# thangktran/HardwareAwareOptimalQuantumCircuitCuttingAndKnitting

Hardware: AMD Instinct MI355X
Metric: subcircuit-instances/s (full-knit wall time = ms_per_step), syc 32 p=2 (higher is better)
Workload: dtype f64

## Files before the change

hardwareawareoptimalquantumcircuitcuttingandknitting_amd/_lib.py:

```python
from __future__ import annotations

import ctypes
import os
import threading

_HERE = os.path.dirname(os.path.abspath(__file__))
LIB_PATH = os.environ.get("QKNIT_LIB") or os.path.join(_HERE, "libqknit.so")

c_i32, c_i64, c_u32, c_u64 = ctypes.c_int32, ctypes.c_int64, ctypes.c_uint32, ctypes.c_uint64
c_vp, c_dp, c_lp = ctypes.c_void_p, ctypes.POINTER(ctypes.c_double), ctypes.POINTER(ctypes.c_int64)


class QkPass(ctypes.Structure):
    _fields_ = [("tile_mask", c_u64), ("group_begin", c_i32), ("group_end", c_i32),
                ("flags", c_i32), ("traced_local", c_u32)]


class QkProgram(ctypes.Structure):
    _fields_ = [("n", c_i32), ("n_eff", c_i32), ("m", c_i32), ("n_slots", c_i32),
                ("packed", c_i32), ("n_passes", c_i32), ("passes", ctypes.POINTER(QkPass)),
                ("ops", c_vp), ("groups", c_vp), ("mats", c_vp)]


class QkLowrankPlan(ctypes.Structure):
    _fields_ = [("nbits", c_i32), ("terms", c_i32), ("rows_a", c_i64), ("rows_b", c_i64), ("mask_a", c_u64),
                ("mask_b", c_u64), ("wt_a", c_vp), ("wt_b", c_vp), ("probes", c_vp), ("lam_tol", ctypes.c_double),
                ("s_tol", ctypes.c_double), ("s_abs", ctypes.c_double), ("rank_tol", ctypes.c_double),
                ("rank_tol_rel", ctypes.c_double)]


class QkKnitPlan(ctypes.Structure):
    _fields_ = [("n_frag", c_i32), ("nbits", c_i32), ("terms", c_i64), ("rows", ctypes.POINTER(c_i64)),
                ("clbit_masks", ctypes.POINTER(c_u64)), ("transforms", ctypes.POINTER(c_vp))]


SIGNATURES = {
    "qk_version": (ctypes.c_char_p, []),
    "qk_ctx_create": (c_i32, [ctypes.c_int, ctypes.POINTER(c_vp)]),
    "qk_ctx_destroy": (c_i32, [c_vp]),
    "qk_ctx_set_stream": (c_i32, [c_vp, c_vp]),
    "qk_ctx_synchronize": (c_i32, [c_vp]),
    "qk_last_error": (ctypes.c_char_p, [c_vp]),
    "qk_stream_create_cu_masked": (c_i32, [ctypes.c_int, ctypes.POINTER(c_u32), ctypes.c_int, ctypes.POINTER(c_vp)]),
    "qk_stream_destroy": (c_i32, [c_vp]),
    "qk_stream_cu_count": (c_i32, [ctypes.c_int, c_vp, ctypes.POINTER(ctypes.c_int)]),
    "qk_out_alloc": (c_i32, [c_vp, c_i64, ctypes.POINTER(c_vp)]),
    "qk_out_free": (c_i32, [c_vp, c_vp]),
    "qk_out_mapped_bytes": (c_i32, [c_vp, ctypes.POINTER(c_i64)]),
    "qk_out_write_rate": (c_i32, [c_vp, c_vp, c_i64, ctypes.POINTER(ctypes.c_double)]),
    "qk_out_stats": (c_i32, [ctypes.POINTER(c_i64), c_i32]),
    "qk_sweep_workspace_bytes": (c_i32, [ctypes.POINTER(QkProgram), c_i64, ctypes.POINTER(c_i64)]),
    "qk_sweep": (c_i32, [c_vp, ctypes.POINTER(QkProgram), c_i64, c_vp, c_vp, c_vp, c_i64, c_vp]),
    "qk_module_compile": (c_i32, [c_vp, ctypes.c_char_p, ctypes.POINTER(ctypes.c_char_p), ctypes.c_int,
                                  ctypes.POINTER(c_vp)]),
    "qk_module_destroy": (c_i32, [c_vp]),
    "qk_module_load": (c_i32, [c_vp, c_vp, c_i64, ctypes.POINTER(ctypes.c_char_p), ctypes.c_int, ctypes.POINTER(c_vp)]),
    "qk_module_code": (c_i32, [c_vp, c_vp, ctypes.POINTER(c_i64)]),
    "qk_sweep_compiled": (c_i32, [c_vp, c_vp, ctypes.POINTER(QkProgram), c_i64, c_vp, c_vp, c_vp, c_i64,
                                  c_vp]),
    "qk_sweep_compiled_labels": (c_i32, [c_vp, c_vp, ctypes.POINTER(QkProgram), c_i64, c_vp, c_vp, c_i64, c_vp,
                                         c_vp, c_i64, c_vp]),
    "qk_sweep_compiled_multi": (c_i32, [c_vp, c_vp, ctypes.c_int, ctypes.POINTER(QkProgram), c_lp, c_vp, c_vp, c_lp,
                                        c_vp, c_vp, c_lp, c_vp, c_vp]),
    "qk_sweep_compiled_multi_shared": (c_i32, [c_vp, c_vp, ctypes.c_int, ctypes.POINTER(QkProgram), c_lp, c_vp, c_vp,
                                               c_lp, c_vp, c_vp, c_lp, c_vp, c_vp, c_lp, c_vp, c_vp]),
    "qk_reduce_labels": (c_i32, [c_vp, c_i64, c_vp, c_i64, c_vp, c_vp]),
    "qk_gemm_keyed": (c_i32, [c_vp, c_i64, c_i64, c_i64, c_vp, c_i64, c_vp, c_i64, c_vp, c_i64,
                              c_vp, c_i64, c_vp, ctypes.c_int]),
    "qk_gemm_keyed_pred": (c_i32, [c_vp, c_i64, c_i64, c_i64, c_vp, c_i64, c_vp, c_i64, c_vp, c_i64,
                                   c_vp, c_i64, c_vp, ctypes.c_int, c_vp]),
    "qk_gemm_outer_paired": (c_i32, [c_vp, c_i64, c_i64, c_i64, c_vp, c_i64, c_vp, c_i64, c_vp, c_i64,
                                     c_vp, c_vp]),
    "qk_knit_outer_stream": (c_i32, [c_vp, ctypes.c_int, c_i64, c_vp, c_i64, c_vp, c_i64, ctypes.c_uint64,
                                     ctypes.c_uint64, c_vp]),
    "qk_knit_outer_stream_kind": (c_i32, [ctypes.c_int, c_i64, c_u64, c_u64, c_i64, c_i64,
                                          ctypes.POINTER(ctypes.c_int), ctypes.POINTER(ctypes.c_int)]),
    "qk_knit_outer_stream_range": (c_i32, [c_vp, ctypes.c_int, c_i64, c_vp, c_i64, c_vp, c_i64, ctypes.c_uint64,
                                           ctypes.c_uint64, c_i64, c_i64, c_vp, c_vp]),
    "qk_rank_factors": (c_i32, [c_vp, c_i64, c_vp, c_vp, ctypes.c_double, ctypes.c_double, ctypes.c_double,
                                ctypes.c_int, c_vp, c_vp, c_vp]),
    "qk_prep_workspace_bytes": (c_i32, [c_vp, c_i64, c_i64, ctypes.POINTER(c_i64)]),
    "qk_prep_operands": (c_i32, [c_vp, ctypes.c_int, ctypes.c_int, c_vp, c_vp, c_i64, c_i64, c_vp, ctypes.c_int,
                                 c_vp, c_vp, c_i64, c_i64, c_vp, c_vp, c_vp, c_vp, c_vp, c_vp, c_i64]),
    "qk_qprep_workspace_bytes": (c_i32, [c_vp, c_i64, c_i64, ctypes.POINTER(c_i64)]),
    "qk_qprep_grams": (c_i32, [c_vp, ctypes.c_int, ctypes.c_int, c_vp, c_vp, c_i64, c_i64, ctypes.c_int, c_vp, c_vp,
                               c_i64, c_i64, c_vp, c_vp, c_vp, c_vp, c_vp, c_i64]),
    "qk_qprep_compress_check": (c_i32, [c_vp, ctypes.c_int, ctypes.c_int, ctypes.c_int, c_vp, c_vp, c_i64, c_i64,
                                        ctypes.c_int, c_vp, c_vp, c_i64, c_i64, c_vp, c_vp, c_vp, c_vp, c_vp, c_vp,
                                        c_vp, c_vp, ctypes.c_double, ctypes.c_double, c_vp, c_vp, c_vp, c_i64]),
    "qk_compress_operands": (c_i32, [c_vp, ctypes.c_int, ctypes.c_int, c_vp, c_vp, c_i64, c_vp, c_vp, c_vp, c_i64,
                                     c_vp]),
    "qk_compress_operands_ld": (c_i32, [c_vp, ctypes.c_int, ctypes.c_int, c_vp, c_vp, c_i64, c_i64, c_vp, c_i64, c_vp,
                                        c_vp, c_i64, c_i64, c_vp, c_i64]),
    "qk_compress_probe_v": (c_i32, [c_vp, ctypes.c_int, ctypes.c_int, c_vp, c_vp, c_i64, c_i64, c_vp, c_i64, c_vp, c_vp,
                                    c_i64, c_i64, c_vp, c_i64, c_vp, c_i64, c_vp, c_i64]),
    "qk_probe_errors_vpart": (c_i32, [c_vp, ctypes.c_int, ctypes.c_int, c_vp, c_i64, c_i64, c_vp, c_i64, c_vp, c_vp,
                                      c_i64, c_vp, c_vp, ctypes.c_double, ctypes.c_double, c_vp, c_vp, c_vp, c_i64,
                                      c_vp]),
    "qk_probe_workspace_bytes": (c_i32, [c_vp, c_i64, ctypes.POINTER(c_i64)]),
    "qk_probe_errors": (c_i32, [c_vp, ctypes.c_int, ctypes.c_int, c_vp, c_i64, c_i64, c_vp, c_i64, c_vp, c_vp, c_i64,
                                c_i64, c_vp, c_i64, c_vp, c_vp, ctypes.c_double, ctypes.c_double, c_vp, c_vp, c_vp,
                                c_i64]),
    "qk_probe_errors_tally": (c_i32, [c_vp, ctypes.c_int, ctypes.c_int, c_vp, c_i64, c_i64, c_vp, c_i64, c_vp, c_vp, c_i64,
                                c_i64, c_vp, c_i64, c_vp, c_vp, ctypes.c_double, ctypes.c_double, c_vp, c_vp, c_vp,
                                c_i64, c_vp]),
    "qk_probe_accept": (c_i32, [c_vp, c_vp, ctypes.c_int, c_vp, ctypes.c_double, ctypes.c_double, c_vp, c_vp]),
    "qk_rank_tally": (c_i32, [c_vp, c_vp, c_vp, c_vp]),
    "qk_knit_workspace_bytes": (c_i32, [ctypes.POINTER(QkKnitPlan), ctypes.POINTER(c_i64)]),
    "qk_knit": (c_i32, [c_vp, ctypes.POINTER(QkKnitPlan), c_vp, c_vp, c_i64, c_vp]),
    "qk_khatri_rao": (c_i32, [c_vp, c_i64, c_i64, c_i64, c_vp, c_i64, c_vp, c_i64, c_vp]),
    "qk_gather_rows": (c_i32, [c_vp, c_i64, c_i64, c_vp, c_vp, c_vp, c_vp]),
    "qk_npd_workspace_bytes": (c_i32, [c_i64, c_i64, ctypes.POINTER(c_i64)]),
    "qk_threshold_count": (c_i32, [c_vp, c_i64, c_vp, ctypes.c_double, c_vp, c_i64, c_vp]),
    "qk_npd": (c_i32, [c_vp, c_i64, c_vp, ctypes.c_double, c_i64, c_vp, c_i64, c_vp, c_vp, c_vp]),
    "qk_qd_from_rows": (c_i32, [c_vp, c_i64, c_i64, c_vp, c_vp, ctypes.c_double, c_vp]),
    "qk_qd_merge": (c_i32, [c_vp, c_i64, c_vp, c_vp, c_i64, c_vp, c_vp, ctypes.c_double, c_i64, c_vp]),
    "qk_qd_axpby": (c_i32, [c_vp, c_i64, ctypes.c_double, c_vp, ctypes.c_double, c_vp, ctypes.c_double, c_vp]),
    "qk_hellinger": (c_i32, [c_vp, c_i64, c_vp, c_vp, c_vp]),
    "qk_knit_lowrank_workspace_bytes": (c_i32, [c_vp, c_vp, ctypes.POINTER(c_i64)]),
    "qk_knit_lowrank": (c_i32, [c_vp, c_vp, c_vp, c_vp, c_vp, c_i64, c_vp, c_vp]),
    "qk_comm_unique_id": (c_i32, [c_vp]),
    "qk_comm_init": (c_i32, [c_vp, c_vp, ctypes.c_int, ctypes.c_int, ctypes.POINTER(c_vp)]),
    "qk_comm_destroy": (c_i32, [c_vp]),
    "qk_comm_size": (c_i32, [c_vp, ctypes.POINTER(ctypes.c_int), ctypes.POINTER(ctypes.c_int)]),
    "qk_allreduce": (c_i32, [c_vp, c_vp, c_vp, c_vp, c_i64]),
    "qk_reduce": (c_i32, [c_vp, c_vp, c_vp, c_vp, c_i64, ctypes.c_int]),
    "qk_allgather": (c_i32, [c_vp, c_vp, c_vp, c_vp, c_i64]),
    "qk_alltoall": (c_i32, [c_vp, c_vp, c_vp, c_vp, c_i64]),
    "qk_knit_select_workspace_bytes": (c_i32, [ctypes.c_int, c_u64, c_u64, ctypes.POINTER(c_i64)]),
    "qk_knit_select": (c_i32, [c_vp, ctypes.c_int, c_i64, c_vp, c_i64, c_vp, c_i64, c_u64, c_u64, ctypes.c_double,
                               c_vp, c_vp, c_i64, c_i64, c_vp, c_vp, c_vp]),
    "qk_select_above": (c_i32, [c_vp, c_i64, c_vp, ctypes.c_double, c_i64, c_i64, c_vp, c_vp, c_vp]),
    "qk_npd_pairs_workspace_bytes": (c_i32, [c_i64, ctypes.POINTER(c_i64)]),
    "qk_npd_pairs": (c_i32, [c_vp, c_i64, c_vp, c_vp, c_vp, c_i64, c_vp, c_vp, c_vp]),
    "qk_sample_cdf": (c_i32, [c_vp, c_i64, c_vp, c_i64, c_vp, c_vp]),
    "qk_sample_counts": (c_i32, [c_vp, c_i64, c_i64, c_vp, c_vp, c_vp, c_i64, c_vp, c_i64, c_u64, c_vp]),
    "qk_fold_counts": (c_i32, [c_vp, c_i64, c_vp, c_i64, c_vp, c_vp, c_i64, ctypes.c_double, c_vp]),
}

_lock = threading.Lock()
_lib = None


class QknitError(RuntimeError):
    pass


def lib() -> ctypes.CDLL:
    global _lib
    with _lock:
        if _lib is None:
            if not os.path.exists(LIB_PATH):
                raise QknitError(
                    f"{LIB_PATH} not built: run `python -c 'import __graft_entry__ as g; g.build()'`"
                )
            handle = ctypes.CDLL(LIB_PATH)
            for name, (res, args) in SIGNATURES.items():
                fn = getattr(handle, name)
                fn.restype = res
                fn.argtypes = args
            _lib = handle
        return _lib


def check(ctx, status: int, what: str) -> None:
    if status != 0:
        msg = lib().qk_last_error(ctx)
        raise QknitError(f"{what} failed (status {status}): {msg.decode() if msg else ''}")
```

hardwareawareoptimalquantumcircuitcuttingandknitting_amd/csrc/qknit_prep.hip:

```cpp
#include <hip/hip_runtime.h>

#include <cstdint>
#include <string>

#include "internal.h"

namespace {

typedef double d4_t __attribute__((ext_vector_type(4)));
typedef double d2_t __attribute__((ext_vector_type(2)));

constexpr int PK = 64;
constexpr int PCT = 128;
constexpr int PNP = 16;
constexpr int PTH = 512;
constexpr int XLD = PCT + 2;
constexpr int PG_BLK = 10;
constexpr int PPG = PG_BLK * 256;
constexpr int PPA = PPG;
constexpr int PPB = PPG + PK * PNP;
__host__ __device__ constexpr int prep_tri(int bi, int bj) { return bi * 4 - bi * (bi - 1) / 2 + (bj - bi); }

struct PrepSide {
    const double* Wt;
    const double* q;
    int64_t ldq;
    int64_t N;
    int R;
    double* X;
    const double* P;
};

struct PrepArgs {
    PrepSide s[2];
    int K;
    int split;
    double* part;
};

#ifndef QK_PREP_RS
#define QK_PREP_RS 16
#endif
constexpr int PRS = QK_PREP_RS;
constexpr int PRPW = PRS / 8;
static_assert(PRS % 8 == 0 && PRS >= 8, "stage rows: a multiple of 8 (8 waves)");
#ifndef QK_PREP_NS
#define QK_PREP_NS 2
#endif
#ifndef QK_PREP_WG_PER_CU
#define QK_PREP_WG_PER_CU 2
#endif
#ifndef QK_COMPRESS_COLS
#define QK_COMPRESS_COLS 1
#endif
#ifndef QK_PREP_EXP
#define QK_PREP_EXP 0
#endif
constexpr int PNS = QK_PREP_NS;
#ifndef QK_PREP_QPAD
#define QK_PREP_QPAD 16
#endif
#ifndef QK_PREP_WPAD
#define QK_PREP_WPAD 16
#endif
constexpr int QLD = PCT + QK_PREP_QPAD;
constexpr int WLD = PK + QK_PREP_WPAD;
struct PrepStage {
    double q[PRS][QLD];
    double w[PRS][WLD];
};
union PrepLds {
    PrepStage st[PNS];
    double x[PK][XLD];
};

__device__ __forceinline__ void prep_glds(const double* src, double* lds_row) {
    __builtin_amdgcn_global_load_lds(reinterpret_cast<const void*>(src),
                                     reinterpret_cast<__attribute__((address_space(3))) void*>(
                                         reinterpret_cast<uintptr_t>(lds_row)),
                                     16, 0, 0);
}

__device__ __forceinline__ void prep_vmwait(int n) {
    switch (n < 15 ? n : 15) {
#define QK_PW(k) case k: asm volatile("s_waitcnt vmcnt(" #k ")" ::: "memory"); break;
        QK_PW(0) QK_PW(1) QK_PW(2) QK_PW(3) QK_PW(4) QK_PW(5) QK_PW(6) QK_PW(7)
        QK_PW(8) QK_PW(9) QK_PW(10) QK_PW(11) QK_PW(12) QK_PW(13) QK_PW(14) QK_PW(15)
#undef QK_PW
    }
}

__global__ __launch_bounds__(PTH, 2 * QK_PREP_WG_PER_CU) void qk_prep_operands_kernel(PrepArgs a) {
    __shared__ __attribute__((aligned(16))) PrepLds L;
    const int tid = threadIdx.x, lane = tid & 63, wave = tid >> 6;
    const int l16 = lane & 15, l4 = lane >> 4;
    const int K = a.K;
    int gi0, gj0, gi1 = -1, gj1 = -1;
    switch (wave) {
        case 4: gi0 = 0, gj0 = 1, gi1 = 0, gj1 = 2; break;
        case 5: gi0 = 0, gj0 = 3, gi1 = 1, gj1 = 2; break;
        case 6: gi0 = 1, gj0 = 3; break;
        case 7: gi0 = 2, gj0 = 3; break;
        default: gi0 = gj0 = wave; break;
    }
    gi0 = __builtin_amdgcn_readfirstlane(gi0), gj0 = __builtin_amdgcn_readfirstlane(gj0);
    gi1 = __builtin_amdgcn_readfirstlane(gi1), gj1 = __builtin_amdgcn_readfirstlane(gj1);
    const int wave_s = __builtin_amdgcn_readfirstlane(wave);
    for (int sd = 0; sd < 2; ++sd) {
        const PrepSide& S = a.s[sd];
        const int R = S.R;
        const int nst = (R + PRS - 1) / PRS;
        const int64_t tiles = S.N / PCT;
        d4_t g0 = {0, 0, 0, 0}, g1 = {0, 0, 0, 0}, u = {0, 0, 0, 0};
        const bool mine = !a.split || (int)(blockIdx.x & 1) == sd;
        const int64_t t_first = a.split ? (int64_t)(blockIdx.x >> 1) : (int64_t)blockIdx.x;
        const int64_t t_step = a.split ? (int64_t)(gridDim.x >> 1) : (int64_t)gridDim.x;
        for (int64_t t = mine ? t_first : tiles; t < tiles; t += t_step) {
            const int64_t c0 = t * PCT;
            int nload[PNS];
            auto issue = [&](int st) {
                PrepStage& P = L.st[st % PNS];
                int n = 0;
#pragma unroll
                for (int h = 0; h < PRPW; ++h) {
                    const int rl = PRPW * wave_s + h, r = st * PRS + rl;
                    if (r < R) {
                        prep_glds(S.q + (int64_t)r * S.ldq + c0 + 2 * lane, &P.q[rl][0]);
                        ++n;
                        if (2 * lane < K) prep_glds(S.Wt + (int64_t)r * K + 2 * lane, &P.w[rl][0]);
                        ++n;
                    }
                }
                nload[st % PNS] = n;
            };
            asm volatile("s_waitcnt lgkmcnt(0)" ::: "memory");
            __builtin_amdgcn_s_barrier();
            for (int st = 0; st < PNS - 1 && st < nst; ++st) issue(st);
            d4_t x[4];
#pragma unroll
            for (int i = 0; i < 4; ++i) x[i] = (d4_t){0, 0, 0, 0};
            for (int st = 0; st < ((QK_PREP_EXP & 4) ? 0 : nst); ++st) {
                int after = 0;
                for (int d = st + 1; d < st + PNS - 1 && d < nst; ++d) after += nload[d % PNS];
                prep_vmwait(after);
                asm volatile("s_waitcnt lgkmcnt(0)" ::: "memory");
                __builtin_amdgcn_s_barrier();
                const PrepStage& P = L.st[st % PNS];
                double qb[PRS / 4], wa[PRS / 4][4];
#pragma unroll
                for (int kk = 0; kk < PRS / 4; ++kk) {
                    const int rl = 4 * kk + l4;
                    const bool rv = st * PRS + rl < R;
                    qb[kk] = rv ? P.q[rl][16 * wave + l16] : 0.0;
#pragma unroll
                    for (int i = 0; i < 4; ++i) {
                        const int k = 16 * i + l16;
                        wa[kk][i] = (rv && k < K) ? P.w[rl][k] : 0.0;
                    }
                }
                if (st + PNS - 1 < nst) issue(st + PNS - 1);
#pragma unroll
                for (int kk = 0; kk < PRS / 4; ++kk)
#pragma unroll
                    for (int i = 0; i < 4; ++i) x[i] = __builtin_amdgcn_mfma_f64_16x16x4f64(wa[kk][i], qb[kk], x[i], 0, 0, 0);
            }
            const bool probes = S.P != nullptr && wave < 4;
            constexpr int PPB = 8;
            const double* pp = probes ? S.P + (int64_t)l16 * S.N + c0 + l4 : nullptr;
            double pxn[PPB];
#pragma unroll
            for (int j = 0; j < PPB; ++j) pxn[j] = probes ? pp[4 * j] : 0.0;
            asm volatile("s_waitcnt lgkmcnt(0)" ::: "memory");
            __builtin_amdgcn_s_barrier();
#pragma unroll
            for (int i = 0; i < 4; ++i)
#pragma unroll
                for (int rr = 0; rr < 4; ++rr) L.x[16 * i + l4 + 4 * rr][16 * wave + l16] = x[i][rr];
            asm volatile("s_waitcnt lgkmcnt(0)" ::: "memory");
            __builtin_amdgcn_s_barrier();
            for (int s8 = 0; s8 < ((QK_PREP_EXP & 1) ? 0 : PCT / 4); s8 += PPB) {
                double px[PPB];
#pragma unroll
                for (int j = 0; j < PPB; ++j) px[j] = pxn[j];
                if (probes && s8 + PPB < PCT / 4) {
#pragma unroll
                    for (int j = 0; j < PPB; ++j) pxn[j] = pp[4 * (s8 + PPB + j)];
                }
                if (wave < 4) {
#pragma unroll
                    for (int j = 0; j < PPB; ++j) {
                        const double av = L.x[16 * gi0 + l16][4 * (s8 + j) + l4];
                        g0 = __builtin_amdgcn_mfma_f64_16x16x4f64(av, av, g0, 0, 0, 0);
                        if (probes) u = __builtin_amdgcn_mfma_f64_16x16x4f64(av, px[j], u, 0, 0, 0);
                    }
                } else {
#pragma unroll
                    for (int j = 0; j < PPB; ++j) {
                        const int c = 4 * (s8 + j) + l4;
                        const double a0 = L.x[16 * gi0 + l16][c];
                        const double b0 = L.x[16 * gj0 + l16][c];
                        g0 = __builtin_amdgcn_mfma_f64_16x16x4f64(a0, b0, g0, 0, 0, 0);
                        if (gi1 >= 0) {
                            const double a1 = gi1 == gi0 ? a0 : L.x[16 * gi1 + l16][c];
                            const double b1 = L.x[16 * gj1 + l16][c];
                            g1 = __builtin_amdgcn_mfma_f64_16x16x4f64(a1, b1, g1, 0, 0, 0);
                        }
                    }
                }
            }
            if (!(QK_PREP_EXP & 2)) {
                d2_t z[8];
#pragma unroll
                for (int v = 0; v < 8; ++v) z[v] = *reinterpret_cast<const d2_t*>(&L.x[8 * wave_s + v][2 * lane]);
#pragma unroll
                for (int v = 0; v < 8; ++v)
                    if (8 * wave_s + v < K) *reinterpret_cast<d2_t*>(S.X + (int64_t)(8 * wave_s + v) * S.N + c0 + 2 * lane) = z[v];
            }
        }
        double* p = sd == 0 ? a.part + (int64_t)blockIdx.x * PPA
                            : a.part + (int64_t)gridDim.x * PPA + (int64_t)blockIdx.x * PPB;
#pragma unroll
        for (int rr = 0; rr < 4; ++rr) {
            const int e = (l4 + 4 * rr) * 16 + l16;
            p[prep_tri(gi0, gj0) * 256 + e] = g0[rr];
            if (gi1 >= 0) p[prep_tri(gi1, gj1) * 256 + e] = g1[rr];
            if (sd == 1 && wave < 4) p[PPG + (16 * wave + l4 + 4 * rr) * PNP + l16] = u[rr];
        }
    }
}

constexpr int PRW = 16;
__global__ __launch_bounds__(64 * PRW) void qk_prep_reduce_kernel(const double* __restrict__ part, int nblk,
                                                                  int K, double* __restrict__ GA,
                                                                  double* __restrict__ GB, double* __restrict__ U) {
    __shared__ double acc[PRW][64];
    const int lane = threadIdx.x & 63, grp = threadIdx.x >> 6;
    const int e = blockIdx.x * 64 + lane;
    int sd = -1, off = 0;
    double* dst = nullptr;
    double* mirror = nullptr;
    if (e < 2 * PPG) {
        sd = e < PPG ? 0 : 1;
        off = e - sd * PPG;
        const int blk = off >> 8;
        const int bi = blk < 4 ? 0 : blk < 7 ? 1 : blk < 9 ? 2 : 3;
        const int bj = bi + blk - prep_tri(bi, bi);
        const int r = 16 * bi + ((off >> 4) & 15), c = 16 * bj + (off & 15);
        if (r < K && c < K) {
            double* G = sd == 0 ? GA : GB;
            dst = G + r * K + c;
            if (bi != bj) mirror = G + c * K + r;
        }
    } else if (e < 2 * PPG + PNP * K) {
        const int f = e - 2 * PPG;
        sd = 1, off = PPG + f, dst = U + f;
    }
    if (!dst) sd = -1;
    double s = 0.0;
    if (sd >= 0) {
        const int PPART = sd == 0 ? PPA : PPB;
        const double* p = part + (sd == 0 ? 0 : (int64_t)nblk * PPA) + off;
        double t[8] = {0, 0, 0, 0, 0, 0, 0, 0};
        int b = grp;
        for (; b + 31 * PRW < nblk; b += 32 * PRW) {
            double v[32];
#pragma unroll
            for (int u = 0; u < 32; ++u) v[u] = p[(int64_t)(b + PRW * u) * PPART];
#pragma unroll
            for (int u = 0; u < 32; ++u) t[u & 7] += v[u];
        }
        for (; b < nblk; b += PRW) t[0] += p[(int64_t)b * PPART];
        s = ((t[0] + t[1]) + (t[2] + t[3])) + ((t[4] + t[5]) + (t[6] + t[7]));
    }
    acc[grp][lane] = s;
    __syncthreads();
    if (grp == 0 && dst) {
        double v[PRW];
#pragma unroll
        for (int w = 0; w < PRW; ++w) v[w] = acc[w][lane];
#pragma unroll
        for (int h = PRW / 2; h >= 1; h >>= 1)
#pragma unroll
            for (int w = 0; w < h; ++w) v[w] += v[w + h];
        *dst = v[0];
        if (mirror) *mirror = v[0];
    }
}

__global__ __launch_bounds__(256) void qk_compress_kernel(int K, int rmax, const double* __restrict__ TA,
                                                          const double* __restrict__ XA, int64_t NA, int64_t ldxa,
                                                          double* __restrict__ A2, int64_t lda2,
                                                          const double* __restrict__ TB,
                                                          const double* __restrict__ XB, int64_t NB, int64_t ldxb,
                                                          double* __restrict__ B2, int64_t ldb2) {
    __shared__ double T[8][PK];
    __shared__ double part[4][8][64];
    const bool bs = blockIdx.y == 1;
    const double* Tg = bs ? TB : TA;
    const double* X = bs ? XB : XA;
    double* out = bs ? B2 : A2;
    const int64_t N = bs ? NB : NA, ld = bs ? ldxb : ldxa, ldo = bs ? ldb2 : lda2;
    const int l = threadIdx.x & 63;
    const int q = __builtin_amdgcn_readfirstlane(threadIdx.x >> 6);
    auto load = [&](int64_t c0, double (&xv)[16]) {
        const int64_t c = c0 + l;
#pragma unroll
        for (int u = 0; u < 16; ++u) {
            const int k = 16 * q + u;
            const double* row = X + (int64_t)k * ld;
            xv[u] = (k < K && c < N) ? row[c] : 0.0;
        }
    };
    double xv[16];
    int64_t c0 = (int64_t)blockIdx.x * 64;
    if (c0 < N) load(c0, xv);
    {
        const int n = rmax * K, e0 = threadIdx.x, e1 = threadIdx.x + 256;
// ... 188 lines not shown
#pragma unroll
        for (int s0 = 0; s0 < 32; s0 += VB) {
            double pb[VB];
#pragma unroll
            for (int s = 0; s < VB; ++s) {
                const int64_t col = base + 4 * (s0 + s) + k4;
                pb[s] = col < N ? pr[col] : 0.0;
            }
#pragma unroll
            for (int s = 0; s < VB; ++s) {
                const double a = i16 < 8 ? Bt[wave][i16][4 * (s0 + s) + k4] : 0.0;
                va = __builtin_amdgcn_mfma_f64_16x16x4f64(a, pb[s], va, 0, 0, 0);
            }
        }
    }
#pragma unroll
    for (int r = 0; r < 2; ++r) Vw[wave][(k4 + 4 * r) * 16 + i16] = va[r];
    __syncthreads();
    if (tid < PV_PART)
        vpart[wg * PV_PART + tid] = (Vw[0][tid] + Vw[1][tid]) + (Vw[2][tid] + Vw[3][tid]);
}

__global__ __launch_bounds__(256) void qk_probe_v_kernel(int rmax, const double* __restrict__ B2, int64_t ldb2,
                                                         int64_t NB, const double* __restrict__ P, int64_t ldp,
                                                         double* __restrict__ vpart) {
    const int tid = threadIdx.x, lane = tid & 63, wave = tid >> 6;
    double acc[8][4];
#pragma unroll
    for (int jj = 0; jj < 8; ++jj)
#pragma unroll
        for (int q = 0; q < 4; ++q) acc[jj][q] = 0.0;
    struct Col {
        double b[8], pv[4];
    };
    const int64_t step = (int64_t)gridDim.x * 64;
    auto fetch = [&](int64_t c, Col& x) {
        const int64_t cc = c < NB ? c : NB - 1;
#pragma unroll
        for (int jj = 0; jj < 8; ++jj) x.b[jj] = B2[(int64_t)min(jj, rmax - 1) * ldb2 + cc];
#pragma unroll
        for (int q = 0; q < 4; ++q) x.pv[q] = P[(int64_t)(4 * wave + q) * ldp + cc];
    };
    auto mac = [&](const Col& x) {
#pragma unroll
        for (int jj = 0; jj < 8; ++jj)
#pragma unroll
            for (int q = 0; q < 4; ++q) acc[jj][q] = fma(x.b[jj], x.pv[q], acc[jj][q]);
    };
    int64_t c = (int64_t)blockIdx.x * 64 + lane;
    if (c < NB) {
        Col x0, x1;
        fetch(c, x0);
        for (;; c += 2 * step) {
            fetch(c + step, x1);
            __builtin_amdgcn_sched_barrier(0);
            mac(x0);
            if (c + step >= NB) break;
            fetch(c + 2 * step, x0);
            __builtin_amdgcn_sched_barrier(0);
            mac(x1);
            if (c + 2 * step >= NB) break;
        }
    }
#pragma unroll
    for (int jj = 0; jj < 8; ++jj)
#pragma unroll
        for (int q = 0; q < 4; ++q) {
            double v = acc[jj][q];
#pragma unroll
            for (int s = 1; s < 64; s <<= 1) v += __shfl_xor(v, s, 64);
            acc[jj][q] = jj < rmax ? v : 0.0;
        }
    double* out = vpart + (int64_t)blockIdx.x * PV_PART;
    if (lane < 32) {
        const int j8 = lane >> 2, q = lane & 3;
        double v = 0.0;
#pragma unroll
        for (int jj = 0; jj < 8; ++jj)
#pragma unroll
            for (int qq = 0; qq < 4; ++qq)
                if (jj == j8 && qq == q) v = acc[jj][qq];
        out[j8 * 16 + 4 * wave + q] = v;
    }
}

__global__ __launch_bounds__(256) void qk_probe_d_kernel(int K, int rmax, const double* __restrict__ XA, int64_t ldx,
                                                         int64_t NA, const double* __restrict__ A2, int64_t lda2,
                                                         const double* __restrict__ U,
                                                         const double* __restrict__ vpart, int gv,
                                                         double* __restrict__ epart) {
    __shared__ double Us[PK][PNP];
    __shared__ double Vs[16][PNP];
    __shared__ double ep[4][2 * PNP];
    const int tid = threadIdx.x, lane = tid & 63, wave = tid >> 6, l16 = lane & 15, l4 = lane >> 4;
    {
        __shared__ double vh[PV_PART];
        const int e = tid & (PV_PART - 1), h = tid >> 7;
        double t[16];
#pragma unroll
        for (int u = 0; u < 16; ++u) t[u] = 0.0;
        int b = h;
        for (; b + 30 < gv; b += 32) {
            double v[16];
#pragma unroll
            for (int u = 0; u < 16; ++u) v[u] = vpart[(int64_t)(b + 2 * u) * PV_PART + e];
#pragma unroll
            for (int u = 0; u < 16; ++u) t[u] += v[u];
        }
        for (; b < gv; b += 2) t[0] += vpart[(int64_t)b * PV_PART + e];
#pragma unroll
        for (int w = 8; w >= 1; w >>= 1)
#pragma unroll
            for (int u = 0; u < w; ++u) t[u] += t[u + w];
        if (h == 1) vh[e] = t[0];
        __syncthreads();
        if (h == 0) Vs[e / 16][e % 16] = -(t[0] + vh[e]);
        else Vs[8 + e / 16][e % 16] = 0.0;
    }
    for (int e = tid; e < PK * PNP; e += 256) Us[e / PNP][e % PNP] = (e / PNP) < K ? U[e] : 0.0;
    __syncthreads();
    double e2 = 0.0, f2 = 0.0;
    for (int64_t cb = (int64_t)blockIdx.x * 4 + wave; cb * 16 < NA; cb += (int64_t)gridDim.x * 4) {
        const int64_t c = cb * 16 + l16;
        double av[PK / 4], a2[2];
#pragma unroll
        for (int kk = 0; kk < PK / 4; ++kk) av[kk] = XA[(int64_t)min(4 * kk + l4, K - 1) * ldx + c];
#pragma unroll
        for (int jj = 0; jj < 2; ++jj) a2[jj] = A2[(int64_t)min(4 * jj + l4, rmax - 1) * lda2 + c];
        d4_t acc = {0, 0, 0, 0};
#pragma unroll
        for (int kk = 0; kk < PK / 4; ++kk)
            acc = __builtin_amdgcn_mfma_f64_16x16x4f64(av[kk], Us[4 * kk + l4][l16], acc, 0, 0, 0);
#pragma unroll
        for (int rr = 0; rr < 4; ++rr) f2 = fma(acc[rr], acc[rr], f2);
#pragma unroll
        for (int jj = 0; jj < 2; ++jj)
            acc = __builtin_amdgcn_mfma_f64_16x16x4f64(a2[jj], Vs[4 * jj + l4][l16], acc, 0, 0, 0);
#pragma unroll
        for (int rr = 0; rr < 4; ++rr) e2 = fma(acc[rr], acc[rr], e2);
    }
    e2 += __shfl_xor(e2, 16, 64);
    e2 += __shfl_xor(e2, 32, 64);
    f2 += __shfl_xor(f2, 16, 64);
    f2 += __shfl_xor(f2, 32, 64);
    if (l4 == 0) {
        ep[wave][l16] = e2;
        ep[wave][PNP + l16] = f2;
    }
    __syncthreads();
    if (tid < 2 * PNP)
        epart[(int64_t)blockIdx.x * 2 * PNP + tid] = ep[0][tid] + ep[1][tid] + ep[2][tid] + ep[3][tid];
}

constexpr int PE = 2 * PNP;

__global__ __launch_bounds__(256) void qk_probe_accept_kernel(const double* __restrict__ epart, int n,
                                                              const int32_t* __restrict__ r_dev, double tol,
                                                              double rel_tol, double* __restrict__ e2_out,
                                                              int32_t* __restrict__ k_out, double* __restrict__ err_out,
                                                              int64_t* __restrict__ tally = nullptr) {
    __shared__ double acc[256];
    const int tid = threadIdx.x, p = tid % PE;
    constexpr int STEP = 256 / PE;
    double s8[8] = {0, 0, 0, 0, 0, 0, 0, 0};
    int b = tid / PE;
    for (; b + 31 * STEP < n; b += 32 * STEP) {
        double v[32];
#pragma unroll
        for (int u = 0; u < 32; ++u) v[u] = epart[(int64_t)(b + u * STEP) * PE + p];
#pragma unroll
        for (int u = 0; u < 32; ++u) s8[u & 7] += v[u];
    }
    for (; b < n; b += STEP) s8[0] += epart[(int64_t)b * PE + p];
    const double s = ((s8[0] + s8[1]) + (s8[2] + s8[3])) + ((s8[4] + s8[5]) + (s8[6] + s8[7]));
    acc[tid] = s;
    __syncthreads();
    for (int w = 128; w >= PE; w >>= 1) {
        if (tid < w) acc[tid] += acc[tid + w];
        __syncthreads();
    }
    if (tid < PE && e2_out) e2_out[tid] = acc[tid];
    if (tid == 0 && k_out) {
        double m = 0.0, f = 0.0;
        for (int q = 0; q < PNP; ++q) {
            m = fmax(m, acc[q]);
            f = fmax(f, acc[PNP + q]);
        }
        const double err = sqrt(m);
        const double bound = fmax(tol, rel_tol * sqrt(f));
        const int r = *r_dev;
        if (err_out) *err_out = err;
        const int k = (r > 0 && err <= bound) ? r : 0;
        *k_out = k;
        if (tally) {
            tally[0] += r == 0 ? 1 : 0;
            tally[1] += (r > 0 && k == 0) ? 1 : 0;
            tally[2] = k;
            tally[3] += 1;
        }
    }
}

constexpr int QG_T = 512;
constexpr int QG_LD = PCT + 18;
constexpr int QG_NB = 5;
constexpr int QG_RMAX = 16 * QG_NB;
constexpr int QG_UP = QG_NB * (QG_NB + 1) / 2;
constexpr int QG_PART = (QG_UP + QG_NB) * 256;

template <typename F>
__device__ __forceinline__ void stage16(const double* __restrict__ src, int n, int nthreads, F store) {
    for (int e0 = threadIdx.x; e0 < n; e0 += 16 * nthreads) {
        double v[16];
#pragma unroll
        for (int u = 0; u < 16; ++u) {
            const int e = e0 + u * nthreads;
            v[u] = e < n ? src[e] : 0.0;
        }
#pragma unroll
        for (int u = 0; u < 16; ++u) {
            const int e = e0 + u * nthreads;
            if (e < n) store(e, v[u]);
        }
    }
}

struct QGramSide {
    const double* q;
    int64_t ldq, N;
    int R;
    const double* P;
};

struct QGramArgs {
    QGramSide s[2];
    int split;
    int slots;
    double* part;
};

__device__ __forceinline__ void qg_block(int b, int& bi, int& bj) {
    bi = 0;
    int n = QG_NB;
    while (b >= n) {
        b -= n;
        ++bi;
        --n;
    }
    bj = bi + b;
}

__global__ __launch_bounds__(QG_T, 2) void qk_qgram_kernel(QGramArgs a) {
    extern __shared__ __attribute__((aligned(16))) double qs[];
    const int tid = threadIdx.x, lane = tid & 63, wave = tid >> 6;
    const int l16 = lane & 15, l4 = lane >> 4;
    const int wave_s = __builtin_amdgcn_readfirstlane(wave);
    for (int sd = 0; sd < 2; ++sd) {
        const QGramSide& S = a.s[sd];
        const int R = S.R, nb = (R + 15) / 16;
        int bi[3], bj[3];
        bool live[3], probe[3];
#pragma unroll
        for (int t = 0; t < 3; ++t) {
            const int b = wave + 8 * t;
            probe[t] = b >= QG_UP;
            if (!probe[t]) qg_block(b, bi[t], bj[t]);
            else bi[t] = b - QG_UP, bj[t] = 0;
            live[t] = b < QG_UP + QG_NB && bi[t] < nb && (probe[t] ? S.P != nullptr : bj[t] < nb);
        }
        d4_t acc[3];
#pragma unroll
        for (int t = 0; t < 3; ++t) acc[t] = (d4_t){0, 0, 0, 0};
        const bool mine = !a.split || (int)(blockIdx.x & 1) == sd;
        const int64_t t_first = a.split ? (int64_t)(blockIdx.x >> 1) : (int64_t)blockIdx.x;
        const int64_t t_step = a.split ? (int64_t)(gridDim.x >> 1) : (int64_t)gridDim.x;
        const int64_t tiles = S.N / PCT;
        const bool want_p = (live[0] && probe[0]) || (live[1] && probe[1]) || (live[2] && probe[2]);
        for (int64_t t = mine ? t_first : tiles; t < tiles; t += t_step) {
            const int64_t c0 = t * PCT;
            asm volatile("s_waitcnt lgkmcnt(0)" ::: "memory");
            __builtin_amdgcn_s_barrier();
            for (int r = wave_s; r < R; r += QG_T / 64) prep_glds(S.q + (int64_t)r * S.ldq + c0 + 2 * lane, &qs[r * QG_LD]);
            d2_t pv[PCT / 8];
            if (want_p) {
                const double* pp = S.P + (int64_t)l16 * S.N + c0 + 2 * l4;
#pragma unroll
                for (int s8 = 0; s8 < PCT / 8; ++s8) pv[s8] = *reinterpret_cast<const d2_t*>(pp + 8 * s8);
            }
            asm volatile("s_waitcnt vmcnt(0)" ::: "memory");
            __builtin_amdgcn_s_barrier();
#pragma unroll
            for (int t3 = 0; t3 < 3; ++t3) {
                if (!live[t3]) continue;
                const int ra = 16 * bi[t3] + l16, rb = 16 * bj[t3] + l16;
                const d2_t* xa = reinterpret_cast<const d2_t*>(&qs[(ra < R ? ra : R - 1) * QG_LD + 2 * l4]);
                const d2_t* xb = reinterpret_cast<const d2_t*>(&qs[(rb < R ? rb : R - 1) * QG_LD + 2 * l4]);
                const double ma = ra < R ? 1.0 : 0.0, mb = rb < R ? 1.0 : 0.0;
                d4_t g = acc[t3];
                if (probe[t3]) {
#pragma unroll
                    for (int s8 = 0; s8 < PCT / 8; ++s8) {
                        const d2_t x = xa[4 * s8];
                        g = __builtin_amdgcn_mfma_f64_16x16x4f64(ma * x.x, pv[s8].x, g, 0, 0, 0);
                        g = __builtin_amdgcn_mfma_f64_16x16x4f64(ma * x.y, pv[s8].y, g, 0, 0, 0);
                    }
                } else {
// ... 200 lines not shown
                const d2_t x = buf[ch & 1][u];
#pragma unroll
                for (int j = 0; j < 8; ++j) {
                    const double m = w * Mt[i < R ? i : R - 1][j];
                    acc[j].x = fma(m, x.x, acc[j].x);
                    acc[j].y = fma(m, x.y, acc[j].y);
                }
            }
        }
        __syncthreads();
#pragma unroll
        for (int j = 0; j < 8; ++j) {
            if (j < rmax) *reinterpret_cast<d2_t*>(B2 + (int64_t)j * N + c) = acc[j];
            *reinterpret_cast<d2_t*>(&b2s[j][2 * tid]) = acc[j];
        }
#pragma unroll
        for (int u = 0; u < PNP * QB_COLS / 2 / QB_T; ++u) {
            const int e = tid + u * QB_T, p = e / (QB_COLS / 2), cc = 2 * (e % (QB_COLS / 2));
            *reinterpret_cast<d2_t*>(&ps[p][cc]) = pvv[u];
        }
        __syncthreads();
        const int h0 = vhalf * (QB_COLS / 2);
        double v0 = 0.0, v1 = 0.0;
        for (int cc = h0; cc < h0 + QB_COLS / 2; cc += 2) {
            v0 = fma(b2s[vj][cc], ps[vp][cc], v0);
            v1 = fma(b2s[vj][cc + 1], ps[vp][cc + 1], v1);
        }
        vacc += v0 + v1;
    }
    if (vhalf) vh[vj * PNP + vp] = vacc;
    __syncthreads();
    if (!vhalf) vpart[(int64_t)blockIdx.x * QV_PART + vj * PNP + vp] = vj < rmax ? vacc + vh[vj * PNP + vp] : 0.0;
}

__global__ __launch_bounds__(QA_T) void qk_qcompress_a_kernel(int K, int rmax, int R, const double* __restrict__ T,
                                                              const double* __restrict__ Wt, const double* __restrict__ q,
                                                              int64_t ldq, int64_t N, const double* __restrict__ U,
                                                              const double* __restrict__ vpart, int gv,
                                                              double* __restrict__ A2, double* __restrict__ epart) {
    __shared__ double Mt[QG_RMAX][8];
    __shared__ double Zt[QG_RMAX][PNP];
    __shared__ double Vs[8][PNP];
    __shared__ double red[QA_T / 64][2 * PNP];
    __shared__ QcStage st;
    const int tid = threadIdx.x, lane = tid & 63, wave = tid >> 6;
    const int64_t c = (int64_t)blockIdx.x * QA_COLS + 2 * tid;
    {
        const int e = tid;
        double t8[8] = {0, 0, 0, 0, 0, 0, 0, 0};
        int b = 0;
        for (; b + 31 < gv; b += 32) {
            double v[32];
#pragma unroll
            for (int u = 0; u < 32; ++u) v[u] = vpart[(int64_t)(b + u) * QV_PART + e];
#pragma unroll
            for (int u = 0; u < 32; ++u) t8[u & 7] += v[u];
        }
        for (; b < gv; ++b) t8[0] += vpart[(int64_t)b * QV_PART + e];
        Vs[e / PNP][e % PNP] = ((t8[0] + t8[1]) + (t8[2] + t8[3])) + ((t8[4] + t8[5]) + (t8[6] + t8[7]));
    }
    qc_stage(K, rmax, R, T, Wt, U, st, Mt, Zt, QA_T);
    __syncthreads();
    d2_t a2[8], ref[PNP];
#pragma unroll
    for (int j = 0; j < 8; ++j) a2[j] = (d2_t){0.0, 0.0};
#pragma unroll
    for (int p = 0; p < PNP; ++p) ref[p] = (d2_t){0.0, 0.0};
    d2_t buf[2][QC_CH];
    auto load = [&](int ch, d2_t (&bb)[QC_CH]) {
#pragma unroll
        for (int u = 0; u < QC_CH; ++u) {
            const int i = min(ch * QC_CH + u, R - 1);
            bb[u] = *reinterpret_cast<const d2_t*>(q + (int64_t)i * ldq + c);
        }
    };
    const int nch = (R + QC_CH - 1) / QC_CH;
    load(0, buf[0]);
#pragma unroll
    for (int ch = 0; ch < QG_RMAX / QC_CH; ++ch) {
        if (ch >= nch) break;
        if (ch + 1 < nch) load(ch + 1, buf[(ch + 1) & 1]);
#pragma unroll
        for (int u = 0; u < QC_CH; ++u) {
            const int i = ch * QC_CH + u;
            const double w = i < R ? 1.0 : 0.0;
            const int ii = i < R ? i : R - 1;
            const d2_t x = buf[ch & 1][u];
            const d2_t xw = (d2_t){w * x.x, w * x.y};
#pragma unroll
            for (int j = 0; j < 8; ++j) {
                const double m = Mt[ii][j];
                a2[j].x = fma(m, xw.x, a2[j].x);
                a2[j].y = fma(m, xw.y, a2[j].y);
            }
#pragma unroll
            for (int p = 0; p < PNP; ++p) {
                const double z = Zt[ii][p];
                ref[p].x = fma(z, xw.x, ref[p].x);
                ref[p].y = fma(z, xw.y, ref[p].y);
            }
        }
    }
#pragma unroll
    for (int j = 0; j < 8; ++j)
        if (j < rmax) *reinterpret_cast<d2_t*>(A2 + (int64_t)j * N + c) = a2[j];
    double e2[PNP], f2[PNP];
#pragma unroll
    for (int p = 0; p < PNP; ++p) {
        d2_t d = ref[p];
#pragma unroll
        for (int j = 0; j < 8; ++j) {
            d.x = fma(-a2[j].x, Vs[j][p], d.x);
            d.y = fma(-a2[j].y, Vs[j][p], d.y);
        }
        e2[p] = fma(d.x, d.x, d.y * d.y);
        f2[p] = fma(ref[p].x, ref[p].x, ref[p].y * ref[p].y);
    }
#pragma unroll
    for (int p = 0; p < PNP; ++p) {
#pragma unroll
        for (int s = 1; s < 64; s <<= 1) {
            e2[p] += __shfl_xor(e2[p], s, 64);
            f2[p] += __shfl_xor(f2[p], s, 64);
        }
    }
    if (lane == 0) {
#pragma unroll
        for (int p = 0; p < PNP; ++p) {
            red[wave][p] = e2[p];
            red[wave][PNP + p] = f2[p];
        }
    }
    __syncthreads();
    if (tid < 2 * PNP) epart[(int64_t)blockIdx.x * PE + tid] = red[0][tid] + red[1][tid];
}

int probe_grid_d(qk_ctx* ctx, int64_t NA) {
    const int64_t blocks = (NA + 63) / 64;
    const int64_t cap = (int64_t)(ctx->cus > 0 ? ctx->cus : 256) * 2;
    return (int)(blocks < cap ? (blocks > 0 ? blocks : 1) : cap);
}

int fail(qk_ctx* ctx, int code, const char* msg) {
    ctx->err = msg;
    return code;
}

#ifndef QK_PREP_SPLIT
#define QK_PREP_SPLIT 1
#endif
bool prep_split(qk_ctx* ctx, int64_t NA, int64_t NB) {
    const int64_t tiles = (NA > NB ? NA : NB) / PCT;
    const int64_t g = (int64_t)(ctx->cus > 0 ? ctx->cus : 256) * QK_PREP_WG_PER_CU;
    return QK_PREP_SPLIT && tiles > 0 && 2 * tiles <= g;
}

int prep_grid(qk_ctx* ctx, int64_t NA, int64_t NB) {
    const int64_t tiles = (NA > NB ? NA : NB) / PCT;
    if (prep_split(ctx, NA, NB)) return (int)(2 * tiles);
    const int64_t g = (int64_t)(ctx->cus > 0 ? ctx->cus : 256) * QK_PREP_WG_PER_CU;
    return (int)(tiles < g ? (tiles > 0 ? tiles : 1) : g);
}

}

extern "C" {

int qk_prep_workspace_bytes(qk_ctx* ctx, int64_t NA, int64_t NB, int64_t* bytes) {
    if (!ctx || !bytes) return QK_EARG;
    *bytes = (int64_t)prep_grid(ctx, NA, NB) * (PPA + PPB) * (int64_t)sizeof(double);
    return QK_OK;
}

int qk_prep_operands(qk_ctx* ctx, int K, int RA, const double* WtA, const double* qA, int64_t ldqA, int64_t NA,
                     double* XA, int RB, const double* WtB, const double* qB, int64_t ldqB, int64_t NB, double* XB,
                     const double* probes, double* GA, double* GB, double* U, double* work, int64_t work_bytes) {
    if (!ctx) return QK_EARG;
    if (K < 2 || K > PK || (K & 1) || RA < 1 || RB < 1)
        return fail(ctx, QK_EARG, "qk_prep_operands: need even 2 <= K <= 64 and R >= 1 on both sides");
    if (((reinterpret_cast<uintptr_t>(WtA) | reinterpret_cast<uintptr_t>(WtB) | reinterpret_cast<uintptr_t>(qA) |
          reinterpret_cast<uintptr_t>(qB)) & 15) || (ldqA & 1) || (ldqB & 1))
        return fail(ctx, QK_EARG, "qk_prep_operands: 16-B aligned Wt / q and even ldq required");
    if (NA < PCT || NB < PCT || NA % PCT || NB % PCT || ldqA < NA || ldqB < NB)
        return fail(ctx, QK_EARG, "qk_prep_operands: columns must be a positive multiple of 128 (ldq >= N)");
    if (!WtA || !qA || !XA || !WtB || !qB || !XB || !probes || !GA || !GB || !U || !work)
        return fail(ctx, QK_EARG, "qk_prep_operands: null buffer");
    const int G = prep_grid(ctx, NA, NB);
    if (work_bytes < (int64_t)G * (PPA + PPB) * (int64_t)sizeof(double))
        return fail(ctx, QK_EARG, "qk_prep_operands: workspace too small (qk_prep_workspace_bytes)");
    if (hipSetDevice(ctx->device) != hipSuccess) return fail(ctx, QK_EHIP, "qk_prep_operands: hipSetDevice");
    PrepArgs args;
    args.s[0] = PrepSide{WtA, qA, ldqA, NA, RA, XA, nullptr};
    args.s[1] = PrepSide{WtB, qB, ldqB, NB, RB, XB, probes};
    args.K = K;
    args.split = prep_split(ctx, NA, NB) ? 1 : 0;
    args.part = work;
    hipLaunchKernelGGL(qk_prep_operands_kernel, dim3(G), dim3(PTH), 0, ctx->stream, args);
    const int outs = 2 * PPG + PNP * K;
    hipLaunchKernelGGL(qk_prep_reduce_kernel, dim3((outs + 63) / 64), dim3(64 * PRW), 0, ctx->stream, work, G, K, GA,
                       GB, U);
    const hipError_t e = hipGetLastError();
    if (e != hipSuccess) return fail(ctx, QK_EHIP, (std::string("qk_prep_operands: ") + hipGetErrorString(e)).c_str());
    return QK_OK;
}

int qk_qprep_workspace_bytes(qk_ctx* ctx, int64_t NA, int64_t NB, int64_t* bytes) {
    if (!ctx || !bytes) return QK_EARG;
    const int G = prep_grid(ctx, NA, NB);
    const int64_t gb = (NB + QB_SPAN - 1) / QB_SPAN, ga = (NA + QA_COLS - 1) / QA_COLS;
    const int64_t grams = (int64_t)2 * G * QG_PART + 2 * QG_RMAX * QG_RMAX + QG_RMAX * PNP;
    const int64_t check = gb * QV_PART + ga * PE;
    *bytes = (grams > check ? grams : check) * (int64_t)sizeof(double);
    return QK_OK;
}

int qk_qprep_grams(qk_ctx* ctx, int K, int RA, const double* WtA, const double* qA, int64_t ldqA, int64_t NA, int RB,
                   const double* WtB, const double* qB, int64_t ldqB, int64_t NB, const double* probes, double* GA,
                   double* GB, double* U, double* work, int64_t work_bytes) {
    if (!ctx) return QK_EARG;
    if (K < 1 || K > PK || RA < 1 || RB < 1 || RA > QG_RMAX || RB > QG_RMAX)
        return fail(ctx, QK_EARG, "qk_qprep_grams: need 1 <= K <= 64 and 1 <= R <= 80 on both sides");
    if (((reinterpret_cast<uintptr_t>(qA) | reinterpret_cast<uintptr_t>(qB) | reinterpret_cast<uintptr_t>(probes)) & 15) ||
        (ldqA & 1) || (ldqB & 1))
        return fail(ctx, QK_EARG, "qk_qprep_grams: 16-B aligned q / probes and even ldq required");
    if (NA < PCT || NB < PCT || NA % PCT || NB % PCT || ldqA < NA || ldqB < NB)
        return fail(ctx, QK_EARG, "qk_qprep_grams: columns must be a positive multiple of 128 (ldq >= N)");
    if (!WtA || !qA || !WtB || !qB || !probes || !GA || !GB || !U || !work)
        return fail(ctx, QK_EARG, "qk_qprep_grams: null buffer");
    int64_t need = 0;
    qk_qprep_workspace_bytes(ctx, NA, NB, &need);
    if (work_bytes < need) return fail(ctx, QK_EARG, "qk_qprep_grams: workspace too small (qk_qprep_workspace_bytes)");
    if (hipSetDevice(ctx->device) != hipSuccess) return fail(ctx, QK_EHIP, "qk_qprep_grams: hipSetDevice");
    const int G = prep_grid(ctx, NA, NB);
    QGramArgs args;
    args.s[0] = QGramSide{qA, ldqA, NA, RA, nullptr};
    args.s[1] = QGramSide{qB, ldqB, NB, RB, probes};
    args.split = prep_split(ctx, NA, NB) ? 1 : 0;
    args.slots = args.split ? G / 2 : G;
    args.part = work;
    double* gq = work + (int64_t)2 * G * QG_PART;
    const size_t lds = (size_t)(RA > RB ? RA : RB) * QG_LD * sizeof(double);
    hipLaunchKernelGGL(qk_qgram_kernel, dim3(G), dim3(QG_T), lds, ctx->stream, args);
    hipLaunchKernelGGL(qk_qgram_reduce_kernel, dim3((2 * QG_PART + 63) / 64), dim3(64 * PRW), 0, ctx->stream, work,
                       args.slots, gq);
    hipLaunchKernelGGL(qk_qproject_kernel, dim3(2 * QP_CB + 1), dim3(256), 0, ctx->stream, K, RA, WtA, RB, WtB, gq, GA,
                       GB, U);
    const hipError_t e = hipGetLastError();
    if (e != hipSuccess) return fail(ctx, QK_EHIP, (std::string("qk_qprep_grams: ") + hipGetErrorString(e)).c_str());
    return QK_OK;
}

int qk_qprep_compress_check(qk_ctx* ctx, int K, int rmax, int RA, const double* WtA, const double* qA, int64_t ldqA,
                            int64_t NA, int RB, const double* WtB, const double* qB, int64_t ldqB, int64_t NB,
                            const double* TA, const double* TB, const double* U, const double* probes, double* A2,
                            double* B2, double* e2, const int32_t* r_dev, double tol, double rel_tol, int32_t* k_out,
                            double* err_out, double* work, int64_t work_bytes) {
    if (!ctx) return QK_EARG;
    if (K < 1 || K > PK || rmax < 1 || rmax > 8 || RA < 1 || RB < 1 || RA > QG_RMAX || RB > QG_RMAX)
        return fail(ctx, QK_EARG, "qk_qprep_compress_check: need 1 <= K <= 64, 1 <= rmax <= 8, 1 <= R <= 80");
    if (NA % QA_COLS || NB % QB_COLS || NA < QA_COLS || NB < QB_COLS || ldqA < NA || ldqB < NB || (ldqA & 1) || (ldqB & 1))
        return fail(ctx, QK_EARG, "qk_qprep_compress_check: column counts must be positive multiples of 512");
    if (((reinterpret_cast<uintptr_t>(qA) | reinterpret_cast<uintptr_t>(qB) | reinterpret_cast<uintptr_t>(A2) |
          reinterpret_cast<uintptr_t>(B2) | reinterpret_cast<uintptr_t>(probes)) & 15))
        return fail(ctx, QK_EARG, "qk_qprep_compress_check: 16-B aligned buffers required");
    if (!WtA || !qA || !WtB || !qB || !TA || !TB || !U || !probes || !A2 || !B2 || !work || (k_out && !r_dev))
        return fail(ctx, QK_EARG, "qk_qprep_compress_check: null buffer");
    const int64_t gb = (NB + QB_SPAN - 1) / QB_SPAN, ga = NA / QA_COLS;
    if (work_bytes < (gb * QV_PART + ga * PE) * (int64_t)sizeof(double))
        return fail(ctx, QK_EARG, "qk_qprep_compress_check: workspace too small (qk_qprep_workspace_bytes)");
    if (hipSetDevice(ctx->device) != hipSuccess) return fail(ctx, QK_EHIP, "qk_qprep_compress_check: hipSetDevice");
    double* vpart = work;
    double* epart = work + gb * QV_PART;
    hipLaunchKernelGGL(qk_qcompress_b_kernel, dim3((unsigned)gb), dim3(QB_T), 0, ctx->stream, K, rmax, RB, TB, WtB, qB,
                       ldqB, NB, probes, B2, vpart);
    hipLaunchKernelGGL(qk_qcompress_a_kernel, dim3((unsigned)ga), dim3(QA_T), 0, ctx->stream, K, rmax, RA, TA, WtA, qA,
                       ldqA, NA, U, vpart, (int)gb, A2, epart);
    hipLaunchKernelGGL(qk_probe_accept_kernel, dim3(1), dim3(256), 0, ctx->stream, epart, (int)ga, r_dev, tol, rel_tol,
                       e2, k_out, err_out);
    const hipError_t e = hipGetLastError();
    if (e != hipSuccess)
        return fail(ctx, QK_EHIP, (std::string("qk_qprep_compress_check: ") + hipGetErrorString(e)).c_str());
    return QK_OK;
}

int qk_compress_operands(qk_ctx* ctx, int K, int rmax, const double* TA, const double* XA, int64_t NA, double* A2,
                         const double* TB, const double* XB, int64_t NB, double* B2) {
    return qk_compress_operands_ld(ctx, K, rmax, TA, XA, NA, NA, A2, NA, TB, XB, NB, NB, B2, NB);
}

int qk_compress_operands_ld(qk_ctx* ctx, int K, int rmax, const double* TA, const double* XA, int64_t NA, int64_t ldxa,
                            double* A2, int64_t lda2, const double* TB, const double* XB, int64_t NB, int64_t ldxb,
                            double* B2, int64_t ldb2) {
    if (!ctx) return QK_EARG;
    if (K < 1 || K > PK || rmax < 1 || rmax > 8 || NA < 1 || NB < 1)
        return fail(ctx, QK_EARG, "qk_compress_operands: need 1 <= K <= 64, 1 <= rmax <= 8, N >= 1");
    if (ldxa < NA || lda2 < NA || ldxb < NB || ldb2 < NB)
        return fail(ctx, QK_EARG, "qk_compress_operands: leading dimension below the width");
    if (!TA || !XA || !A2 || !TB || !XB || !B2) return fail(ctx, QK_EARG, "qk_compress_operands: null buffer");
    if (hipSetDevice(ctx->device) != hipSuccess) return fail(ctx, QK_EHIP, "qk_compress_operands: hipSetDevice");
    const int64_t N = NA > NB ? NA : NB;
    const bool cols = QK_COMPRESS_COLS && NA % 2 == 0 && NB % 2 == 0 && ldxa % 2 == 0 && lda2 % 2 == 0 &&
                      ldxb % 2 == 0 && ldb2 % 2 == 0 &&
                      !((reinterpret_cast<uintptr_t>(XA) | reinterpret_cast<uintptr_t>(XB) |
                         reinterpret_cast<uintptr_t>(A2) | reinterpret_cast<uintptr_t>(B2)) & 15);
    if (cols) {
        hipLaunchKernelGGL(qk_compress_cols_kernel, dim3((unsigned)((N + 127) / 128), 2), dim3(64), 0, ctx->stream, K,
                           rmax, TA, XA, NA, ldxa, A2, lda2, TB, XB, NB, ldxb, B2, ldb2);
    } else {
        int64_t gx = (N + 63) / 64;
        const int64_t cap = (int64_t)(ctx->cus > 0 ? ctx->cus : 256) * 4;
        gx = gx < cap ? gx : cap;
        hipLaunchKernelGGL(qk_compress_kernel, dim3((unsigned)gx, 2), dim3(256), 0, ctx->stream, K, rmax, TA, XA, NA,
                           ldxa, A2, lda2, TB, XB, NB, ldxb, B2, ldb2);
    }
    const hipError_t e = hipGetLastError();
    if (e != hipSuccess)
        return fail(ctx, QK_EHIP, (std::string("qk_compress_operands: ") + hipGetErrorString(e)).c_str());
    return QK_OK;
}

int qk_compress_probe_v(qk_ctx* ctx, int K, int rmax, const double* TA, const double* XA, int64_t NA, int64_t ldxa,
                        double* A2, int64_t lda2, const double* TB, const double* XB, int64_t NB, int64_t ldxb,
                        double* B2, int64_t ldb2, const double* probes, int64_t ldp, double* vpart,
                        int64_t vpart_doubles) {
    if (!ctx) return QK_EARG;
    if (K < 1 || K > PK || rmax < 1 || rmax > 8 || NA < 2 || NB < 2 || (NA | NB | ldxa | lda2 | ldxb | ldb2) & 1)
        return fail(ctx, QK_EARG, "qk_compress_probe_v: need 1 <= K <= 64, 1 <= rmax <= 8, even widths and strides");
    if (ldxa < NA || lda2 < NA || ldxb < NB || ldb2 < NB || ldp < NB)
        return fail(ctx, QK_EARG, "qk_compress_probe_v: leading dimension below the width");
    if (!TA || !XA || !A2 || !TB || !XB || !B2 || !probes || !vpart)
        return fail(ctx, QK_EARG, "qk_compress_probe_v: null buffer");
    if ((reinterpret_cast<uintptr_t>(XA) | reinterpret_cast<uintptr_t>(XB) | reinterpret_cast<uintptr_t>(A2) |
         reinterpret_cast<uintptr_t>(B2)) & 15)
        return fail(ctx, QK_EARG, "qk_compress_probe_v: operands must be 16-B aligned");
    const int64_t ga = (NA + CV_COLS - 1) / CV_COLS, gb = (NB + CV_COLS - 1) / CV_COLS;
    if (vpart_doubles < gb * PV_PART) return fail(ctx, QK_EARG, "qk_compress_probe_v: vpart too small");
    if (hipSetDevice(ctx->device) != hipSuccess) return fail(ctx, QK_EHIP, "qk_compress_probe_v: hipSetDevice");
    hipLaunchKernelGGL(qk_compress_v_kernel, dim3((unsigned)(ga + gb)), dim3(256), 0, ctx->stream, K, rmax, TA, XA, NA,
                       ldxa, A2, lda2, TB, XB, NB, ldxb, B2, ldb2, probes, ldp, vpart, (int)ga);
    const hipError_t e = hipGetLastError();
    if (e != hipSuccess)
        return fail(ctx, QK_EHIP, (std::string("qk_compress_probe_v: ") + hipGetErrorString(e)).c_str());
    return QK_OK;
}

int qk_probe_errors_vpart(qk_ctx* ctx, int K, int rmax, const double* XA, int64_t ldx, int64_t NA, const double* A2,
                          int64_t lda2, const double* U, const double* vpart, int64_t gv, double* e2,
                          const int32_t* r_dev, double tol, double rel_tol, int32_t* k_out, double* err_out,
                          double* work, int64_t work_bytes, int64_t* tally) {
    if (!ctx) return QK_EARG;
    if (K < 1 || K > PK || rmax < 1 || rmax > 8 || NA < 16 || NA % 16 || gv < 1)
        return fail(ctx, QK_EARG, "qk_probe_errors_vpart: need 1 <= K <= 64, 1 <= rmax <= 8, NA % 16 == 0, gv >= 1");
    if (!XA || !A2 || !U || !vpart || !work || (k_out && !r_dev) || (tally && !k_out))
        return fail(ctx, QK_EARG, "qk_probe_errors_vpart: null buffer");
    if (ldx < NA) return fail(ctx, QK_EARG, "qk_probe_errors_vpart: leading dimension");
    const int gd = probe_grid_d(ctx, NA);
    if (work_bytes < (int64_t)(PV_GRID * PV_PART + gd * PE) * (int64_t)sizeof(double))
        return fail(ctx, QK_EARG, "qk_probe_errors_vpart: workspace too small (qk_probe_workspace_bytes)");
    if (hipSetDevice(ctx->device) != hipSuccess) return fail(ctx, QK_EHIP, "qk_probe_errors_vpart: hipSetDevice");
    double* epart = work + PV_GRID * PV_PART;
    hipLaunchKernelGGL(qk_probe_d_kernel, dim3(gd), dim3(256), 0, ctx->stream, K, rmax, XA, ldx, NA, A2, lda2, U, vpart,
                       (int)gv, epart);
    hipLaunchKernelGGL(qk_probe_accept_kernel, dim3(1), dim3(256), 0, ctx->stream, epart, gd, r_dev, tol, rel_tol, e2,
                       k_out, err_out, tally);
    const hipError_t e = hipGetLastError();
    if (e != hipSuccess)
        return fail(ctx, QK_EHIP, (std::string("qk_probe_errors_vpart: ") + hipGetErrorString(e)).c_str());
    return QK_OK;
}

int qk_probe_workspace_bytes(qk_ctx* ctx, int64_t NA, int64_t* bytes) {
    if (!ctx || !bytes) return QK_EARG;
    *bytes = (int64_t)(PV_GRID * PV_PART + probe_grid_d(ctx, NA) * PE) * (int64_t)sizeof(double);
    return QK_OK;
}

int qk_probe_errors(qk_ctx* ctx, int K, int rmax, const double* XA, int64_t ldx, int64_t NA, const double* A2,
                    int64_t lda2, const double* U, const double* B2, int64_t ldb2, int64_t NB, const double* probes,
                    int64_t ldp, double* e2, const int32_t* r_dev, double tol, double rel_tol, int32_t* k_out,
                    double* err_out, double* work, int64_t work_bytes) {
    return qk_probe_errors_tally(ctx, K, rmax, XA, ldx, NA, A2, lda2, U, B2, ldb2, NB, probes, ldp, e2, r_dev, tol,
                                 rel_tol, k_out, err_out, work, work_bytes, nullptr);
}

int qk_probe_errors_tally(qk_ctx* ctx, int K, int rmax, const double* XA, int64_t ldx, int64_t NA, const double* A2,
                          int64_t lda2, const double* U, const double* B2, int64_t ldb2, int64_t NB,
                          const double* probes, int64_t ldp, double* e2, const int32_t* r_dev, double tol,
                          double rel_tol, int32_t* k_out, double* err_out, double* work, int64_t work_bytes,
                          int64_t* tally) {
    if (!ctx) return QK_EARG;
    if (K < 1 || K > PK || rmax < 1 || rmax > 8 || NA < 16 || NA % 16 || NB < 4 || NB % 4)
        return fail(ctx, QK_EARG, "qk_probe_errors: need 1 <= K <= 64, 1 <= rmax <= 8, NA % 16 == 0, NB % 4 == 0");
    if (!XA || !A2 || !U || !B2 || !probes || !work || (k_out && !r_dev) || (tally && !k_out))
        return fail(ctx, QK_EARG, "qk_probe_errors: null buffer");
    if (ldx < NA || ldb2 < NB || ldp < NB) return fail(ctx, QK_EARG, "qk_probe_errors: leading dimension");
    const int gd = probe_grid_d(ctx, NA);
    if (work_bytes < (int64_t)(PV_GRID * PV_PART + gd * PE) * (int64_t)sizeof(double))
        return fail(ctx, QK_EARG, "qk_probe_errors: workspace too small (qk_probe_workspace_bytes)");
    if (hipSetDevice(ctx->device) != hipSuccess) return fail(ctx, QK_EHIP, "qk_probe_errors: hipSetDevice");
    double* vpart = work;
    double* epart = work + PV_GRID * PV_PART;
    hipLaunchKernelGGL(qk_probe_v_kernel, dim3(PV_GRID), dim3(256), 0, ctx->stream, rmax, B2, ldb2, NB, probes, ldp,
                       vpart);
    hipLaunchKernelGGL(qk_probe_d_kernel, dim3(gd), dim3(256), 0, ctx->stream, K, rmax, XA, ldx, NA, A2, lda2, U, vpart,
                       PV_GRID, epart);
    hipLaunchKernelGGL(qk_probe_accept_kernel, dim3(1), dim3(256), 0, ctx->stream, epart, gd, r_dev, tol, rel_tol, e2,
                       k_out, err_out, tally);
    const hipError_t e = hipGetLastError();
    if (e != hipSuccess) return fail(ctx, QK_EHIP, (std::string("qk_probe_errors: ") + hipGetErrorString(e)).c_str());
    return QK_OK;
}

__global__ __launch_bounds__(64) void qk_rank_tally_kernel(const int32_t* __restrict__ r, const int32_t* __restrict__ k,
                                                          int64_t* __restrict__ acc) {
    if (threadIdx.x == 0) {
        const int rv = *r, kv = *k;
        acc[0] += rv == 0 ? 1 : 0;
        acc[1] += (rv > 0 && kv == 0) ? 1 : 0;
        acc[2] = kv;
        acc[3] += 1;
    }
}

int qk_rank_tally(qk_ctx* ctx, const int32_t* r_dev, const int32_t* k_dev, int64_t* acc) {
    if (!ctx) return QK_EARG;
    if (!r_dev || !k_dev || !acc) return fail(ctx, QK_EARG, "qk_rank_tally: null buffer");
    if (hipSetDevice(ctx->device) != hipSuccess) return fail(ctx, QK_EHIP, "qk_rank_tally: hipSetDevice");
    hipLaunchKernelGGL(qk_rank_tally_kernel, dim3(1), dim3(64), 0, ctx->stream, r_dev, k_dev, acc);
    const hipError_t e = hipGetLastError();
    if (e != hipSuccess) return fail(ctx, QK_EHIP, (std::string("qk_rank_tally: ") + hipGetErrorString(e)).c_str());
    return QK_OK;
}

int qk_probe_accept(qk_ctx* ctx, const double* e2, int n, const int32_t* r_dev, double tol, double rel_tol,
                    int32_t* k_out, double* err_out) {
    if (!ctx) return QK_EARG;
    if (!e2 || !r_dev || !k_out || n < 1) return fail(ctx, QK_EARG, "qk_probe_accept: null buffer or n < 1");
    if (hipSetDevice(ctx->device) != hipSuccess) return fail(ctx, QK_EHIP, "qk_probe_accept: hipSetDevice");
    hipLaunchKernelGGL(qk_probe_accept_kernel, dim3(1), dim3(256), 0, ctx->stream, e2, n, r_dev, tol, rel_tol, nullptr,
                       k_out, err_out);
    const hipError_t e = hipGetLastError();
    if (e != hipSuccess) return fail(ctx, QK_EHIP, (std::string("qk_probe_accept: ") + hipGetErrorString(e)).c_str());
    return QK_OK;
}

}
```

hardwareawareoptimalquantumcircuitcuttingandknitting_amd/csrc/qknit_rank.hip:

```cpp
#include <hip/hip_runtime.h>

#include <cmath>

#include "internal.h"

namespace {

constexpr int RK_K = 64;
constexpr int RK_RC = 32;
constexpr int RK_R = 8;
constexpr int RK_THREADS = 128;

#ifdef QK_RANK_DEBUG
__device__ long long qk_rank_dbg[8];
#define RK_STAMP(i) \
    if (threadIdx.x == 0) qk_rank_dbg[i] = wall_clock64();
#else
#define RK_STAMP(i)
#endif

struct RankArgs {
    int K, rmax;
    const double* GA;
    const double* GB;
    double lam_tol, s_tol, s_abs;
    double* TA;
    double* TB;
    int32_t* r_out;
};

template <int CTRL>
__device__ __forceinline__ double dppd(double v) {
    int2 w = *reinterpret_cast<int2*>(&v);
    w.x = __builtin_amdgcn_mov_dpp(w.x, CTRL, 0xF, 0xF, false);
    w.y = __builtin_amdgcn_mov_dpp(w.y, CTRL, 0xF, 0xF, false);
    return *reinterpret_cast<double*>(&w);
}
template <int CTRL>
__device__ __forceinline__ int dppi(int v) {
    return __builtin_amdgcn_mov_dpp(v, CTRL, 0xF, 0xF, false);
}
__device__ __forceinline__ double readlane_d(double v, int l) {
    int2 w = *reinterpret_cast<int2*>(&v);
    w.x = __builtin_amdgcn_readlane(w.x, l);
    w.y = __builtin_amdgcn_readlane(w.y, l);
    return *reinterpret_cast<double*>(&w);
}
constexpr int DPP_XOR1 = 0xB1, DPP_XOR2 = 0x4E, DPP_HALF_MIRROR = 0x141, DPP_MIRROR = 0x140;

__device__ __forceinline__ double rcp_d(double x) {
    const double r = __builtin_amdgcn_rcp(x);
    return fma(r, fma(-x, r, 1.0), r);
}
__device__ __forceinline__ double rsq_d(double x) {
    const double y = __builtin_amdgcn_rsq(x);
    return fma(y * 0.5, fma(-x * y, y, 1.0), y);
}

__device__ __forceinline__ double wsum(double v, int width = 64) {
    if (width >= 2) v += dppd<DPP_XOR1>(v);
    if (width >= 4) v += dppd<DPP_XOR2>(v);
    if (width >= 8) v += dppd<DPP_HALF_MIRROR>(v);
    if (width >= 16) v += dppd<DPP_MIRROR>(v);
    if (width == 32) {
        const double lo = readlane_d(v, 0) + readlane_d(v, 16), hi = readlane_d(v, 32) + readlane_d(v, 48);
        v = (threadIdx.x & 32) ? hi : lo;
    } else if (width == 64) {
        v = (readlane_d(v, 0) + readlane_d(v, 16)) + (readlane_d(v, 32) + readlane_d(v, 48));
    }
    return v;
}

__device__ __forceinline__ void wargmax(double& v, int& idx) {
    auto take = [&](double v2, int i2) {
        if (v2 > v || (v2 == v && i2 < idx)) {
            v = v2;
            idx = i2;
        }
    };
    take(dppd<DPP_XOR1>(v), dppi<DPP_XOR1>(idx));
    take(dppd<DPP_XOR2>(v), dppi<DPP_XOR2>(idx));
    take(dppd<DPP_HALF_MIRROR>(v), dppi<DPP_HALF_MIRROR>(idx));
    take(dppd<DPP_MIRROR>(v), dppi<DPP_MIRROR>(idx));
    double bv = readlane_d(v, 0);
    int bi = __builtin_amdgcn_readlane(idx, 0);
#pragma unroll
    for (int r = 16; r < 64; r += 16) {
        const double v2 = readlane_d(v, r);
        const int i2 = __builtin_amdgcn_readlane(idx, r);
        if (v2 > bv || (v2 == bv && i2 < bi)) {
            bv = v2;
            bi = i2;
        }
    }
    v = bv;
    idx = bi;
}

__global__ __launch_bounds__(RK_THREADS) void qk_rank_factors_kernel(RankArgs a) {
    __shared__ double G[2][RK_K][RK_K + 1];
    __shared__ double L[2][RK_K][RK_RC + 1];
    __shared__ double C[RK_RC][RK_RC + 1];
    __shared__ double Xs[RK_RC][RK_R + 2];
    __shared__ double Ys[RK_RC][RK_R + 2];
    __shared__ double Y[2][RK_R][RK_RC];
    __shared__ int piv[2][RK_RC], nsteps[2], conv[2], rank_s, chol_live[2][2];
    __shared__ double Ts[2][RK_R][RK_K];

    const int tid = threadIdx.x, lane = tid & 63, side = tid >> 6, K = a.K;
    RK_STAMP(0)
    {
        const double* Gs = side ? a.GB : a.GA;
        const int col = lane < K ? lane : K - 1;
        double v[RK_K];
#pragma unroll
        for (int u = 0; u < RK_K; ++u) v[u] = Gs[(u < K ? u : K - 1) * K + col];
#pragma unroll
        for (int u = 0; u < RK_K; ++u)
            if (u < K && lane < K) G[side][u][lane] = v[u];
        __syncthreads();
        RK_STAMP(4)
    }

    double d = lane < K ? G[side][lane][lane] : 0.0;
    bool alive = lane < K;
    double dmax = d;
    {
        int di = lane;
        wargmax(dmax, di);
    }
    bool active = dmax > 0.0, converged = !(dmax > 0.0);
    int steps = 0;
    for (int j = 0; j <= RK_RC; ++j) {
        if (active) {
            const double res = wsum(alive ? fmax(d, 0.0) : 0.0);
            if (res <= a.lam_tol * dmax) {
                converged = true;
                active = false;
            } else if (j == RK_RC) {
                active = false;
            } else {
                double v = alive ? d : -1.0;
                int idx = lane;
                wargmax(v, idx);
                const int p = idx;
                const double dp = v;
                if (!(dp > 0.0)) {
                    active = false;
                } else {
                    double s = lane < K ? 0.5 * (G[side][lane][p] + G[side][p][lane]) : 0.0;
                    for (int i = 0; i < j; ++i) s -= L[side][lane][i] * L[side][p][i];
                    const double col = lane < K ? s / sqrt(dp) : 0.0;
                    if (lane < K) L[side][lane][j] = col;
                    d -= col * col;
                    if (lane == p) {
                        d = 0.0;
                        alive = false;
                        piv[side][j] = p;
                    }
                    steps = j + 1;
                }
            }
        }
        if (lane == 0) chol_live[j & 1][side] = active ? 1 : 0;
        __syncthreads();
        if (!chol_live[j & 1][0] && !chol_live[j & 1][1]) break;
    }
    if (lane == 0) {
        nsteps[side] = steps;
        conv[side] = converged ? 1 : 0;
    }
    __syncthreads();
    const int ra = nsteps[0], rb = nsteps[1];
    bool ok = conv[0] && conv[1] && ra > 0 && rb > 0;
    RK_STAMP(1)

    if (ok) {
        for (int e = tid; e < ra * rb; e += RK_THREADS) {
            const int i = e / rb, j = e % rb;
            double s = 0.0;
            for (int k = 0; k < K; ++k) s += L[0][k][i] * L[1][k][j];
            C[i][j] = s;
        }
    }
    for (int e = tid; e < 2 * RK_R * RK_K; e += RK_THREADS) (&Ts[0][0][0])[e] = 0.0;
    __syncthreads();
    RK_STAMP(2)

    if (side == 0) {
        int r = 0;
        if (ok) {
            const int n = ra * rb;
            const int tmax = (ra < rb ? ra : rb) < a.rmax + 1 ? (ra < rb ? ra : rb) : a.rmax + 1;
            double cut = 0.0;
            for (int t = 0; t < tmax; ++t) {
                double v = -1.0;
                int idx = 1 << 30;
                for (int e = lane; e < n; e += 64) {
                    const double m = fabs(C[e / rb][e % rb]);
                    if (m > v) {
                        v = m;
                        idx = e;
                    }
                }
                wargmax(v, idx);
                if (t == 0) cut = fmax(a.s_tol * v, a.s_abs);
                if (!(v > cut)) break;
                const int pi = idx / rb, pj = idx % rb;
                const double p = C[pi][pj];
                const double sc = 1.0 / sqrt(fabs(p));
                const double xv = lane < ra ? C[lane][pj] * sc : 0.0;
                const double yv = lane < rb ? C[pi][lane] * (p > 0.0 ? sc : -sc) : 0.0;
                if (lane < ra) Xs[lane][t] = xv;
                if (lane < rb) Ys[lane][t] = yv;
                __builtin_amdgcn_fence(__ATOMIC_SEQ_CST, "wavefront");
                __builtin_amdgcn_wave_barrier();
                for (int e = lane; e < n; e += 64) {
                    const int i = e / rb, j = e % rb;
                    C[i][j] = fma(-Xs[i][t], Ys[j][t], C[i][j]);
                }
                __builtin_amdgcn_fence(__ATOMIC_SEQ_CST, "wavefront");
                __builtin_amdgcn_wave_barrier();
                r = t + 1;
            }
            if (r > a.rmax || r > ra) r = 0;
        }
        if (lane == 0) rank_s = r;
    }
    __syncthreads();
    RK_STAMP(5)
    const int r = rank_s;

    if (tid < 2 * r) {
        const int sd = tid / r, t = tid % r;
        const int rx = sd ? rb : ra;
        double* y = Y[sd][t];
        for (int i = rx - 1; i >= 0; --i) {
            double v = sd ? Ys[i][t] : Xs[i][t];
            for (int k = i + 1; k < rx; ++k) v -= L[sd][piv[sd][k]][i] * y[k];
            y[i] = v / L[sd][piv[sd][i]][i];
        }
        for (int i = 0; i < rx; ++i) Ts[sd][t][piv[sd][i]] = y[i];
    }
    __syncthreads();
    for (int e = tid; e < a.rmax * K; e += RK_THREADS) {
        a.TA[e] = Ts[0][e / K][e % K];
        a.TB[e] = Ts[1][e / K][e % K];
    }
    if (tid == 0) *a.r_out = r;
    RK_STAMP(3)
#ifdef QK_RANK_DEBUG
    if (tid == 0) {
        qk_rank_dbg[6] = ra;
        qk_rank_dbg[7] = rb;
    }
#endif
}

}

#ifdef QK_RANK_DEBUG
extern "C" int qk_rank_debug(long long* out) {
    return hipMemcpyFromSymbol(out, HIP_SYMBOL(qk_rank_dbg), sizeof(long long) * 8) == hipSuccess ? 0 : 1;
}
#endif

extern "C" int qk_rank_factors(qk_ctx* ctx, int64_t K, const double* GA, const double* GB, double lam_tol,
                               double s_tol, double s_abs, int rmax, double* TA, double* TB, int32_t* r_out) {
    if (!ctx) return QK_EARG;
    if (K < 1 || K > RK_K || rmax < 1 || rmax > RK_R) {
        ctx->err = "qk_rank_factors: need 1 <= K <= 64 and 1 <= rmax <= 8";
        return QK_EARG;
    }
    if (!GA || !GB || !TA || !TB || !r_out) {
        ctx->err = "qk_rank_factors: null buffer";
        return QK_EARG;
    }
    if (hipSetDevice(ctx->device) != hipSuccess) {
        ctx->err = "qk_rank_factors: hipSetDevice";
        return QK_EHIP;
    }
    RankArgs args{(int)K, rmax, GA, GB, lam_tol, s_tol, s_abs, TA, TB, r_out};
    hipLaunchKernelGGL(qk_rank_factors_kernel, dim3(1), dim3(RK_THREADS), 0, ctx->stream, args);
    const hipError_t e = hipGetLastError();
    if (e != hipSuccess) {
        ctx->err = std::string("qk_rank_factors: ") + hipGetErrorString(e);
        return QK_EHIP;
    }
    return QK_OK;
}
```

hardwareawareoptimalquantumcircuitcuttingandknitting_amd/engine.py:

```python
from __future__ import annotations

import atexit
import contextlib
import ctypes
import dataclasses
import hashlib
import logging
import os
import threading
from dataclasses import dataclass, field
from time import perf_counter

import numpy as np

from . import _lib
from .fragment_program import (FragmentProgram, JobTable, basis_reduce, build_jobs, compile_fragment,
                               dedup_labels)
from .knit_plan import LabelSpace, deposit_keys, factor_vgate
from .sweep_plan import K_SLOT, EncodedProgram, encode

_torch = None


def torch():
# ... 783 lines not shown


def jit_sources(virt, basis: bool = False, relevance: bool = True) -> list:
    from . import sweep_codegen

    frags = prepare_fragments(virt, upload=False, basis=basis, relevance=relevance)
    encs = []
    for fs in frags:
        want, tb, ftb = fs.jit
        dprog = _device_program(fs.prog)[0]
        if fs.dropped or not want or dprog.n <= 12:
            continue
        encs.append(encode(dprog, tile_bits=tb or JIT_TILE_BITS_MAX, final_tile_bits=ftb))
    out = [sweep_codegen.generate(e) for e in encs]
    rounds = max((len(e.passes) for e in encs), default=0)
    if 2 <= len(encs) <= 4 and all(len({e.pass_tile_bits(r) for e in encs if len(e.passes) > r}) == 1
                                   for r in range(rounds)):
        out.append(sweep_codegen.generate_multi(encs))
    return out


def _some_label_unmeasured(prog: FragmentProgram, labels: list) -> bool:
    from .fragment_program import side_branches

    for label in labels:
        if all(len(side_branches(s.endpoint, label[s.vgate_idx])) == 1 for s in prog.slots):
            return True
    return False


def sweep_fragment(ctx: Context, fs: FragmentState, label_range=None):
    T = torch()
    jobs = fs.jobs
    lo, hi = (0, fs.n_rows) if label_range is None else label_range
    width = 1 << fs.prog.m
    if fs.dropped:
        return T.ones((hi - lo, 1), dtype=T.float64, device=T.device("cuda", ctx.device))
    j0, j1 = int(jobs.label_offsets[lo]), int(jobs.label_offsets[hi])
    sub = JobTable(jobs.slot_mats[j0:j1], jobs.sign[j0:j1], jobs.label_offsets[lo : hi + 1] - j0,
                   jobs.branch_bits[j0:j1])
    slot_t, sign_t, off_t = jobs_to_device(sub, ctx.device)
    if sub.n_jobs != hi - lo and fs.dprog.module is not None:
        return fold_traced(ctx, sweep_labels(ctx, fs.dprog, slot_t, sign_t, sub.n_jobs, off_t, hi - lo)[0], fs.fold)
    pjob, _ = sweep_jobs(ctx, fs.dprog, slot_t, sign_t, sub.n_jobs)
    if sub.n_jobs == hi - lo:
        return fold_traced(ctx, pjob, fs.fold)
    return fold_traced(ctx, reduce_labels(ctx, pjob, off_t, hi - lo), fs.fold)


@dataclass
class KnitOperands:

    rows: list
    coefs: list
    transforms: list
    clbits: list
    num_terms: int
    factored_terms: int = 0

    def key_table(self, i: int) -> np.ndarray:
        return deposit_keys(self.clbits[i])


def _affine_stride(clbits: list):
    if not clbits:
        return 0
    c0 = clbits[0]
    return (1 << c0) if list(clbits) == list(range(c0, c0 + len(clbits))) else None


def knit_operands(virt, frags: list[FragmentState], factored: bool = False, compress: bool = True) -> KnitOperands:
    with host_planning():
        return _knit_operands(virt, frags, factored, compress)


def _knit_operands(virt, frags: list[FragmentState], factored: bool, compress: bool) -> KnitOperands:
    vg = [v.operation for v in virt.vgate_instructions]
    space = LabelSpace([g.num_instantiations for g in vg], [g.knit_coefficients() for g in vg])
    clbits = [[] if fs.dropped else list(fs.prog.clbits) for fs in frags]
    if not factored or not vg:
        if any(fs.expand is not None for fs in frags):
            raise ValueError("basis-reduced fragments need the factored knit")
        c = space.coefficients()
        rows, coefs = [], []
        for i, fs in enumerate(frags):
            rows.append(fs.row_of_label()[space.fragment_rows(fs.touches)])
            coefs.append(c if i == 0 else np.ones_like(c))
        return KnitOperands(rows, coefs, [None] * len(frags), clbits, space.num_labels)
    Ts = []
    for j in range(len(vg)):
        eps = _endpoints(virt, j)
        Ts.append(factor_vgate(eps[0], eps[1], vg[j].knit_coefficients()))
    ranks = [t[0].shape[0] for t in Ts]
    transforms = []
    for fs in frags:
        W = np.ones((1, 1))
        sides = _fragment_sides(virt, fs)
        for j in range(len(vg)):
            if sides[j] is None:
                W = np.kron(W, np.ones((ranks[j], 1)))
            else:
                W = np.kron(W, Ts[j][sides[j]])
        if fs.uidx is not None:
            Wu = np.zeros((W.shape[0], len(fs.unique_labels)))
            np.add.at(Wu.T, fs.uidx, W.T)
            W = Wu
        if fs.expand is not None:
            W = W @ fs.expand
        transforms.append(W)
    terms = factored_terms = int(np.prod(ranks))
    if compress and len(frags) == 2 and not any(fs.dropped for fs in frags):
        transforms, terms = _compress_core(transforms, terms)
    return KnitOperands([None] * len(frags), [None] * len(frags), transforms, clbits, terms, factored_terms)


def _compress_core(transforms: list, terms: int, tol: float = 1e-10):
    W0, W1 = transforms
    C = W0.T @ W1
    if C.size == 0:
        return transforms, terms
    U, S, Vt = np.linalg.svd(C, full_matrices=False)
    r = int((S > tol * S[0]).sum()) if S.size and S[0] > 0 else 0
    if r == 0 or r >= terms:
        return transforms, terms
    T0, T1 = np.ascontiguousarray((U[:, :r] * S[:r]).T), np.ascontiguousarray(Vt[:r])
    err = float(np.abs(C - T0.T @ T1).max())
    if not err <= 4 * tol * S[0] + 64 * np.finfo(np.float64).eps * float(np.abs(C).max()):
        return transforms, terms
    return [T0, T1], r


def data_rank_factors(GA: np.ndarray, GB: np.ndarray, **kw):
    from .data_rank import rank_factors

    return rank_factors(GA, GB, **kw)


def rank_factors_device(ctx: Context, GA, GB, rmax: int = 8, out=None):
    from . import data_rank as dr

    T = torch()
    K = GA.shape[0]
    assert GA.shape == (K, K) and GB.shape == (K, K) and GA.is_contiguous() and GB.is_contiguous()
    if out is None:
        out = (T.empty((rmax, K), dtype=T.float64, device=GA.device), T.empty((rmax, K), dtype=T.float64,
                                                                              device=GA.device),
               T.empty(1, dtype=T.int32, device=GA.device))
    TA, TB, r = out
    ctx.check(ctx.lib.qk_rank_factors(ctx.handle, K, GA.data_ptr(), GB.data_ptr(), dr.LAM_TOL, dr.S_TOL, dr.S_ABS,
                                      rmax, TA.data_ptr(), TB.data_ptr(), r.data_ptr()), "qk_rank_factors")
    return TA, TB, r


PREP_COLS = 128
N_PROBES = 16
_PREP_WORK: dict = {}


def prep_ok(K: int, NA: int, NB: int) -> bool:
    return 2 <= K <= 64 and K % 2 == 0 and NA >= PREP_COLS and NB >= PREP_COLS and NA % PREP_COLS == 0 and NB % PREP_COLS == 0


POISON_UNUSED = os.environ.get("QKNIT_POISON_UNUSED", "0") == "1"


def prep_operands(ctx: Context, WtA, qA, WtB, qB, probes, out=None):
    T = torch()
    RA, K = WtA.shape
    RB, K2 = WtB.shape
    assert K == K2 and qA.shape[0] == RA and qB.shape[0] == RB and probes.shape[0] == N_PROBES
    NA, NB = qA.shape[1], qB.shape[1]
    assert probes.shape[1] == NB and all(t.is_contiguous() for t in (WtA, WtB, probes))
    assert qA.stride(1) == 1 and qB.stride(1) == 1
    dev = qA.device
    if out is None:
        gu = T.empty(2 * K * K + K * N_PROBES, dtype=T.float64, device=dev)
        out = (T.empty((K, NA), dtype=T.float64, device=dev), T.empty((K, NB), dtype=T.float64, device=dev),
               gu[:2 * K * K].view(2, K, K), gu[2 * K * K:].view(K, N_PROBES))
    XA, XB, G, U = out
    need = ctypes.c_int64()
    ctx.check(ctx.lib.qk_prep_workspace_bytes(ctx.handle, NA, NB, ctypes.byref(need)), "qk_prep_workspace_bytes")
    key = (str(dev), T.cuda.current_stream(dev).cuda_stream)
    work = _PREP_WORK.get(key)
    if work is None or work.numel() * 8 < need.value:
        work = _PREP_WORK[key] = T.empty(max(need.value // 8, 1), dtype=T.float64, device=dev)
    ctx.check(ctx.lib.qk_prep_operands(ctx.handle, K, RA, WtA.data_ptr(), qA.data_ptr(), qA.stride(0), NA,
                                       XA.data_ptr(), RB, WtB.data_ptr(), qB.data_ptr(), qB.stride(0), NB,
                                       XB.data_ptr(), probes.data_ptr(), G[0].data_ptr(), G[1].data_ptr(),
                                       U.data_ptr(), work.data_ptr(), work.numel() * 8), "qk_prep_operands")
    return XA, XB, G, U


QPREP_ROWS = 80
QPREP = os.environ.get("QKNIT_QPREP", "0") == "1"
_QPREP_WORK: dict = {}


def qprep_ok(K: int, RA: int, RB: int, NA: int, NB: int) -> bool:
    return (QPREP and 1 <= K <= 64 and 1 <= RA <= QPREP_ROWS and 1 <= RB <= QPREP_ROWS and NA >= 512 and NB >= 512
            and NA % 512 == 0 and NB % 512 == 0)


def _qprep_work(ctx: Context, NA: int, NB: int, dev):
    T = torch()
    need = ctypes.c_int64()
    ctx.check(ctx.lib.qk_qprep_workspace_bytes(ctx.handle, NA, NB, ctypes.byref(need)), "qk_qprep_workspace_bytes")
    key = (str(dev), T.cuda.current_stream(dev).cuda_stream)
    work = _QPREP_WORK.get(key)
    if work is None or work.numel() * 8 < need.value:
        work = _QPREP_WORK[key] = T.empty(max(need.value // 8, 1), dtype=T.float64, device=dev)
    return work


def qprep_grams(ctx: Context, WtA, qA, WtB, qB, probes):
    T = torch()
    RA, K = WtA.shape
    RB, K2 = WtB.shape
    assert K == K2 and qA.shape[0] == RA and qB.shape[0] == RB and probes.shape == (N_PROBES, qB.shape[1])
    assert all(t.is_contiguous() for t in (WtA, qA, WtB, qB, probes))
    NA, NB = qA.shape[1], qB.shape[1]
    dev = qA.device
    gu = T.empty(2 * K * K + K * N_PROBES, dtype=T.float64, device=dev)
    G, U = gu[:2 * K * K].view(2, K, K), gu[2 * K * K:].view(K, N_PROBES)
    work = _qprep_work(ctx, NA, NB, dev)
    ctx.check(ctx.lib.qk_qprep_grams(ctx.handle, K, RA, WtA.data_ptr(), qA.data_ptr(), NA, NA, RB, WtB.data_ptr(),
                                     qB.data_ptr(), NB, NB, probes.data_ptr(), G[0].data_ptr(), G[1].data_ptr(),
                                     U.data_ptr(), work.data_ptr(), work.numel() * 8), "qk_qprep_grams")
    return G, U


def qprep_compress_check(ctx: Context, WtA, qA, WtB, qB, TA, TB, U, probes, r, tol: float, rel_tol: float):
    T = torch()
    RA, K = WtA.shape
    RB = WtB.shape[0]
    rmax = TA.shape[0]
    NA, NB = qA.shape[1], qB.shape[1]
    dev = qA.device
    ab = T.empty(rmax * (NA + NB), dtype=T.float64, device=dev)
    A2, B2 = ab[:rmax * NA].view(rmax, NA), ab[rmax * NA:].view(rmax, NB)
    k = T.empty(1, dtype=T.int32, device=dev)
    err = T.empty(1, dtype=T.float64, device=dev)
    work = _qprep_work(ctx, NA, NB, dev)
    ctx.check(ctx.lib.qk_qprep_compress_check(ctx.handle, K, rmax, RA, WtA.data_ptr(), qA.data_ptr(), NA, NA, RB,
                                              WtB.data_ptr(), qB.data_ptr(), NB, NB, TA.data_ptr(), TB.data_ptr(),
                                              U.data_ptr(), probes.data_ptr(), A2.data_ptr(), B2.data_ptr(), None,
                                              r.data_ptr(), tol, rel_tol, k.data_ptr(), err.data_ptr(), work.data_ptr(),
                                              work.numel() * 8), "qk_qprep_compress_check")
    return A2, B2, k, err


def compress_operands(ctx: Context, TA, XA, TB, XB, a_cols: tuple | None = None, a_width: int | None = None):
    T = torch()
    rmax, K = TA.shape
    assert TB.shape == (rmax, K) and XA.shape[0] == K and XB.shape[0] == K
    assert XA.stride(1) == 1 and XB.is_contiguous() and TA.is_contiguous() and TB.is_contiguous()
    NA = XA.shape[1] if a_width is None else a_width
    NB = XB.shape[1]
    ab = T.empty(rmax * (NA + NB), dtype=T.float64, device=XA.device)
    A2 = ab[:rmax * NA].view(rmax, NA)
    B2 = ab[rmax * NA:].view(rmax, NB)
    if a_cols is None:
        assert XA.is_contiguous() and XA.shape[1] == NA
        ctx.check(ctx.lib.qk_compress_operands(ctx.handle, K, rmax, TA.data_ptr(), XA.data_ptr(), NA, A2.data_ptr(),
                                               TB.data_ptr(), XB.data_ptr(), NB, B2.data_ptr()), "qk_compress_operands")
        return A2, B2
    base, n = a_cols
    assert 0 <= base and n >= 1 and base + n <= NA
    src = XA.data_ptr() if XA.shape[1] == n else XA.data_ptr() + 8 * base
    assert XA.shape[1] in (n, NA)
    if POISON_UNUSED:
        A2.fill_(float("nan"))
    ctx.check(ctx.lib.qk_compress_operands_ld(ctx.handle, K, rmax, TA.data_ptr(), src, n, XA.stride(0),
                                              A2.data_ptr() + 8 * base, NA, TB.data_ptr(), XB.data_ptr(), NB, NB,
                                              B2.data_ptr(), NB), "qk_compress_operands_ld")
    return A2, B2


CV_COLS = 512


def compress_probe_v(ctx: Context, TA, XA, TB, XB, probes, a_cols: tuple | None = None, a_width: int | None = None):
    T = torch()
    rmax, K = TA.shape
    assert TB.shape == (rmax, K) and XA.shape[0] == K and XB.shape[0] == K
    assert XA.stride(1) == 1 and XB.is_contiguous() and TA.is_contiguous() and TB.is_contiguous()
    NA = XA.shape[1] if a_width is None else a_width
    NB = XB.shape[1]
    assert probes.is_contiguous() and probes.shape == (N_PROBES, NB)
    ab = T.empty(rmax * (NA + NB), dtype=T.float64, device=XA.device)
    A2 = ab[:rmax * NA].view(rmax, NA)
    B2 = ab[rmax * NA:].view(rmax, NB)
    base, n = (0, NA) if a_cols is None else a_cols
    assert 0 <= base and n >= 1 and base + n <= NA and XA.shape[1] in (n, NA)
    src = XA.data_ptr() if XA.shape[1] == n else XA.data_ptr() + 8 * base
    if a_cols is not None and POISON_UNUSED:
        A2.fill_(float("nan"))
    gv = -(-NB // CV_COLS)
    vpart = T.empty((gv, 8, N_PROBES), dtype=T.float64, device=XA.device)
    ctx.check(ctx.lib.qk_compress_probe_v(ctx.handle, K, rmax, TA.data_ptr(), src, n, XA.stride(0),
                                          A2.data_ptr() + 8 * base, NA, TB.data_ptr(), XB.data_ptr(), NB, NB,
                                          B2.data_ptr(), NB, probes.data_ptr(), NB, vpart.data_ptr(), vpart.numel()),
              "qk_compress_probe_v")
    return A2, B2, vpart


def compress_probe_v_ok(XA, XB, a_cols=None) -> bool:
    n = XA.shape[1] if a_cols is None else a_cols[1]
    base = 0 if a_cols is None or XA.shape[1] == n else a_cols[0]
    return (n % 2 == 0 and XB.shape[1] % 2 == 0 and XA.stride(0) % 2 == 0 and base % 2 == 0
            and (XA.data_ptr() + 8 * base) % 16 == 0 and XB.data_ptr() % 16 == 0)


_PROBE_WORK: dict = {}
def probe_errors(ctx: Context, XA, A2, U, B2, probes, r=None, tol: float = 0.0, a2_cols: tuple | None = None,
                 rel_tol: float = 0.0, tally=None, vpart=None):
    T = torch()
    K, NA = XA.shape
    rmax = A2.shape[0]
    NB = B2.shape[1]
    assert U.shape == (K, N_PROBES) and probes.shape == (N_PROBES, NB) and B2.shape[0] == rmax
    assert all(t.is_contiguous() for t in (A2, U, B2, probes))
    assert XA.stride(1) == 1 and XA.stride(0) >= NA
    off = 0 if a2_cols is None else a2_cols[0]
    assert (a2_cols is None and A2.shape[1] == NA) or (a2_cols is not None and a2_cols[1] == NA)
    dev = XA.device
    need = ctypes.c_int64()
    ctx.check(ctx.lib.qk_probe_workspace_bytes(ctx.handle, NA, ctypes.byref(need)), "qk_probe_workspace_bytes")
    key = (str(dev), T.cuda.current_stream(dev).cuda_stream)
    work = _PROBE_WORK.get(key)
    if work is None or work.numel() * 8 < need.value:
        work = _PROBE_WORK[key] = T.empty(max(need.value // 8, 1), dtype=T.float64, device=dev)
    e2 = T.empty(2 * N_PROBES, dtype=T.float64, device=dev)
    k = T.empty(1, dtype=T.int32, device=dev) if r is not None else None
    err = T.empty(1, dtype=T.float64, device=dev) if r is not None else None
    assert tally is None or (r is not None and tally.dtype == T.int64 and tally.numel() == 4)
    if vpart is not None:
        assert vpart.is_contiguous() and vpart.shape[1:] == (8, N_PROBES)
        ctx.check(ctx.lib.qk_probe_errors_vpart(ctx.handle, K, rmax, XA.data_ptr(), XA.stride(0), NA,
                                                A2.data_ptr() + 8 * off, A2.shape[1], U.data_ptr(), vpart.data_ptr(),
                                                vpart.shape[0], e2.data_ptr(), _ptr(r), tol, rel_tol, _ptr(k), _ptr(err),
                                                work.data_ptr(), work.numel() * 8, _ptr(tally)), "qk_probe_errors_vpart")
        return e2, k, err
    ctx.check(ctx.lib.qk_probe_errors_tally(ctx.handle, K, rmax, XA.data_ptr(), XA.stride(0), NA, A2.data_ptr() + 8 * off,
                                            A2.shape[1], U.data_ptr(), B2.data_ptr(), NB, NB, probes.data_ptr(), NB,
                                            e2.data_ptr(), _ptr(r), tol, rel_tol, _ptr(k), _ptr(err), work.data_ptr(),
                                            work.numel() * 8, _ptr(tally)), "qk_probe_errors_tally")
    return e2, k, err


def probe_accept(ctx: Context, e2, r, tol: float, rel_tol: float = 0.0):
    T = torch()
    k = T.empty(1, dtype=T.int32, device=e2.device)
    err = T.empty(1, dtype=T.float64, device=e2.device)
    ctx.check(ctx.lib.qk_probe_accept(ctx.handle, e2.data_ptr(), 1, r.data_ptr(), tol, rel_tol, k.data_ptr(),
                                      err.data_ptr()), "qk_probe_accept")
    return k, err


def _endpoints(virt, j):
    out = [None, None]
    for instr in virt.circuit:
        op = instr.operation
        if getattr(op, "vgate_idx", None) == j:
            out[op.qubit_idx] = op
    return out


def factored_ok(virt) -> bool:
    frag_of = {}
    for frag in virt.fragment_circuits:
        for q in frag:
            frag_of[q] = frag
    for instr in virt.vgate_instructions:
        a, b = instr.qubits[0], instr.qubits[1]
        if frag_of.get(a) is frag_of.get(b):
            return False
    return True


def _fragment_sides(virt, fs: FragmentState):
    sides = [None] * len(virt.vgate_instructions)
    members = set(fs.fragment)
    for instr in virt.circuit:
        op = instr.operation
        if hasattr(op, "vgate_idx") and instr.qubits[0] in members:
            if sides[op.vgate_idx] is not None:
                raise NotImplementedError("both sides of a virtual gate in one fragment")
            sides[op.vgate_idx] = op.qubit_idx
    return sides


def fragment_operands(ctx: Context, ops: KnitOperands, qs: list) -> list:
    T = torch()
    dev = T.device("cuda", ctx.device)
    mats = []
    for i, q in enumerate(qs):
        q = q.contiguous()
        if ops.transforms[i] is not None:
            W = T.from_numpy(np.ascontiguousarray(ops.transforms[i].T)).to(dev)
            a = T.empty((W.shape[1], q.shape[1]), dtype=T.float64, device=dev)
            gemm_keyed(ctx, W, q, out=a, strideA=q.shape[1])
        else:
            idx_t = T.from_numpy(ops.rows[i]).to(dev)
            coef_t = T.from_numpy(ops.coefs[i]).to(dev)
            a = gather_rows(ctx, q, idx_t, coef_t)
        mats.append(a)
    return mats


def plan_transforms(ops: KnitOperands, frags: list) -> list:
    out = []
    for i, fs in enumerate(frags):
        if ops.transforms[i] is not None:
            out.append(np.ascontiguousarray(ops.transforms[i].T))
            continue
        W = np.zeros((fs.n_rows if not fs.dropped else 1, ops.num_terms))
        W[ops.rows[i], np.arange(ops.num_terms)] = ops.coefs[i]
        out.append(W)
    return out


def knit_plan_c(ctx: Context, virt, frags: list, qs: list, factored: bool = False, out=None):
    T = torch()
    dev = T.device("cuda", ctx.device)
    ops = knit_operands(virt, frags, factored)
    N = virt.circuit.num_clbits
    Ws = [T.from_numpy(W).to(dev) for W in plan_transforms(ops, frags)]
    nf = len(frags)
    rows = (ctypes.c_int64 * nf)(*[W.shape[0] for W in Ws])
    masks = (ctypes.c_uint64 * nf)(*[sum(1 << c for c in cl) for cl in ops.clbits])
    tp = (ctypes.c_void_p * nf)(*[W.data_ptr() for W in Ws])
    plan = _lib.QkKnitPlan(nf, N, ops.num_terms, ctypes.cast(rows, ctypes.POINTER(ctypes.c_int64)),
                           ctypes.cast(masks, ctypes.POINTER(ctypes.c_uint64)),
                           ctypes.cast(tp, ctypes.POINTER(ctypes.c_void_p)))
    need = ctypes.c_int64()
    ctx.check(ctx.lib.qk_knit_workspace_bytes(ctypes.byref(plan), ctypes.byref(need)), "qk_knit_workspace_bytes")
    ws = T.empty(max(need.value, 1), dtype=T.uint8, device=dev)
    if out is None:
        out = T.zeros(1 << N, dtype=T.float64, device=dev)
    qc = [q.contiguous() for q in qs]
    qp = (ctypes.c_void_p * nf)(*[q.data_ptr() for q in qc])
    ctx.check(ctx.lib.qk_knit(ctx.handle, ctypes.byref(plan), qp, ws.data_ptr(), ws.numel(), out.data_ptr()), "qk_knit")
    torch().cuda.current_stream(ctx.device).synchronize()
    return out


def knit_lowrank_c(ctx: Context, pipe, qs: list, out=None, rank_tol: float | None = None,
                   rank_tol_rel: float | None = None):
    from . import data_rank as dr

    T = torch()
    ia, ib = pipe.order[0], pipe.order[-1]
    WA, WB = pipe.transforms[ia], pipe.transforms[ib]
    assert WA is not None and WB is not None, "qk_knit_lowrank needs the factored (transform) knit"
    qa, qb = qs[ia].contiguous(), qs[ib].contiguous()
    probes = pipe._probes(qb.shape[1], qb.device)
    plan = _lib.QkLowrankPlan(pipe.N, WA.shape[1], WA.shape[0], WB.shape[0],
                              sum(1 << c for c in pipe.ops.clbits[ia]), sum(1 << c for c in pipe.ops.clbits[ib]),
                              WA.data_ptr(), WB.data_ptr(), probes.data_ptr(), dr.LAM_TOL, dr.S_TOL, dr.S_ABS,
                              pipe.rank_tol if rank_tol is None else rank_tol,
                              pipe.rank_tol_rel if rank_tol_rel is None else rank_tol_rel)
    need = ctypes.c_int64()
    ctx.check(ctx.lib.qk_knit_lowrank_workspace_bytes(ctx.handle, ctypes.byref(plan), ctypes.byref(need)),
              "qk_knit_lowrank_workspace_bytes")
    ws = T.empty(max(need.value, 1), dtype=T.uint8, device=qa.device)
    if out is None:
        out = T.empty(1 << pipe.N, dtype=T.float64, device=qa.device)
    rank = T.empty(1, dtype=T.int32, device=qa.device)
    ctx.check(ctx.lib.qk_knit_lowrank(ctx.handle, ctypes.byref(plan), qa.data_ptr(), qb.data_ptr(), ws.data_ptr(),
                                      ws.numel(), out.data_ptr(), rank.data_ptr()), "qk_knit_lowrank")
    torch().cuda.current_stream(ctx.device).synchronize()
    return out, rank


class Comm:

    def __init__(self, ctx: Context, uid: bytes, nranks: int, rank: int):
        self.ctx = ctx
        h = ctypes.c_void_p()
        buf = (ctypes.c_uint8 * 128).from_buffer_copy(uid)
        ctx.check(ctx.lib.qk_comm_init(ctx.handle, buf, nranks, rank, ctypes.byref(h)), "qk_comm_init")
        self.handle = h

    @staticmethod
    def unique_id() -> bytes:
        buf = (ctypes.c_uint8 * 128)()
        _lib.check(None, _lib.lib().qk_comm_unique_id(buf), "qk_comm_unique_id")
        return bytes(buf)
# ... 258 lines not shown
```

hardwareawareoptimalquantumcircuitcuttingandknitting_amd/pipeline.py:

```python
from __future__ import annotations

import ctypes
import os
import threading
from time import perf_counter

import numpy as np

from . import _lib, engine
from .fragment_program import JobTable


_PROBES: dict = {}
_PROBES_LOCK = threading.Lock()


def _mm_nt(X, Y):
    L = X.shape[1]
    nb = L // 256 if L % 256 == 0 else 1
    if nb <= 1:
        return X @ Y.T
    Xb = X.view(X.shape[0], nb, 256).transpose(0, 1)
    Yb = Y.reshape(Y.shape[0], nb, 256).transpose(0, 1)
    return (Xb @ Yb.transpose(1, 2)).sum(0)
# ... 88 lines not shown
        items.sort(key=lambda t: (t[0], t[1], t[2]))
        ident = {}
        m = np.fromiter(((f << 56) | (u * bpu + int(perms.get(f, ident.setdefault(bpu, range(bpu)))[t]))
                         for _, f, u, bpu in items for t in range(bpu)), dtype=np.uint64)
        out.append(m)
    return out


XCD_LINE_BITS = 5


def _xcd_tile_order(enc, r: int) -> np.ndarray:
    tm = int(enc.passes[r]["tile_mask"])
    outside = [q for q in range(enc.n) if not (tm >> q) & 1]
    lb = int(os.environ.get("QKNIT_XCD_LINE_BITS", XCD_LINE_BITS))
    low = [i for i, q in enumerate(outside) if q < lb]
    high = [i for i, q in enumerate(outside) if q >= lb]
    bpu = 1 << len(outside)
    if not low or len(high) < 3 or os.environ.get("QKNIT_FINAL_XCD_ORDER", "1") == "0":
        return np.arange(bpu)
    perm = np.zeros(bpu, dtype=np.int64)
    for o in range(bpu):
        t = 0
        for k, i in enumerate(high):
            t |= ((o >> k) & 1) << i
        for k, i in enumerate(low):
            t |= ((o >> (len(high) + k)) & 1) << i
        perm[o] = t
    return perm


def _joined(T, a, b):
    base = a._base
    if (base is not None and b._base is base and base.dim() == 1 and a.is_contiguous() and b.is_contiguous()
            and a.data_ptr() == base.data_ptr()
            and b.data_ptr() == a.data_ptr() + a.numel() * a.element_size()
            and base.numel() == a.numel() + b.numel()):
        return base
    return T.cat([a.reshape(-1), b.reshape(-1)])


class HipBackend:

    def __init__(self, device: int = 0):
        self.T = engine.torch()
        self.device = device
        self.dev = self.T.device("cuda", device)
        self.ctx = engine.get_context(device)

    def prepare_fragments(self, virt, basis: bool = False, jit: bool | None = None, relevance: bool = True):
        return engine.prepare_fragments(virt, self.device, basis=basis, jit=jit, relevance=relevance)

    def upload_jobs(self, jobs: JobTable):
        return engine.jobs_to_device(jobs, self.device)

    def workspace_bytes(self, fs, n_jobs: int) -> int:
        need = ctypes.c_int64()
        self.ctx.check(self.ctx.lib.qk_sweep_workspace_bytes(ctypes.byref(fs.dprog.struct), n_jobs,
                                                             ctypes.byref(need)), "qk_sweep_workspace_bytes")
        return need.value

    def empty(self, shape, dtype):
        return self.T.empty(shape, dtype=dtype, device=self.dev)

    def zeros(self, shape, dtype):
        return self.T.zeros(shape, dtype=dtype, device=self.dev)

    def to_device(self, arr):
        return self.T.from_numpy(np.ascontiguousarray(arr)).to(self.dev)

    def sweep(self, fs, slot, sign, n_jobs, pjob, ws):
        engine.sweep_jobs(self.ctx, fs.dprog, slot, sign, n_jobs, pjob=pjob, workspace=ws)

    def sweep_rows(self, fs):
        return engine.sweep_fragment(self.ctx, fs)

    def fold_traced(self, q, fold):
        return engine.fold_traced(self.ctx, q, fold)

    def device_width(self, fs) -> int:
        return 1 << (fs.dprog.enc.m if fs.dprog is not None else fs.prog.m)

    def bind(self):
        self.ctx.bind_stream()

    def plan_multi(self, frags: list, sweeps: list):
        n = len(frags)
        vp = lambda xs: (ctypes.c_void_p * n)(*xs)
        i64 = lambda xs: (ctypes.c_int64 * n)(*xs)
        module = engine.compiled_multi_module(self.device, [fs.dprog.enc for fs in frags])
        outs = [(sw["q"] if sw["fused"] else sw["pjob"]) for sw in sweeps]
        maps = multi_block_maps([fs.dprog.enc for fs in frags], sweeps)
        self._maps = [None if m is None else self.to_device(m.view(np.int64)) for m in maps]
        rounds = len(maps)
        args = [module, (_lib.QkProgram * n)(*[fs.dprog.struct for fs in frags]), i64([sw["n_jobs"] for sw in sweeps]),
                vp([sw["slot"].data_ptr() for sw in sweeps]), vp([sw["sign"].data_ptr() for sw in sweeps]),
                i64([sw["n_local"] for sw in sweeps]),
                vp([sw["off"].data_ptr() if sw["fused"] else None for sw in sweeps]),
                vp([sw["ws"].data_ptr() for sw in sweeps]), i64([sw["ws"].numel() for sw in sweeps]),
                vp([o.data_ptr() for o in outs]),
                (ctypes.c_void_p * rounds)(*[None if m is None else m.data_ptr() for m in self._maps])]
        shared = [engine.init_prefixes(fs.dprog.enc, sw["jobs"]) if sw.get("jobs") is not None else None
                  for fs, sw in zip(frags, sweeps)]
        self.shared_init = [None if s is None else int(s[0].size) for s in shared]
        if any(s is not None for s in shared):
            self._shared = [None if s is None else (sw["slot"][self.to_device(s[0])].contiguous(),
                                                    self.to_device(s[1]))
                            for s, sw in zip(shared, sweeps)]
            args += [i64([0 if s is None else int(s[0].size) for s in shared]),
                     vp([None if s is None else s[0].data_ptr() for s in self._shared]),
                     vp([None if s is None else s[1].data_ptr() for s in self._shared])]
        return tuple(args)

    def sweep_multi(self, plan):
        module, progs, *rest = plan
        if len(rest) == 12:
            self.ctx.check(self.ctx.lib.qk_sweep_compiled_multi_shared(self.ctx.handle, module, len(progs), progs,
                                                                       *rest), "qk_sweep_compiled_multi_shared")
            return
        self.ctx.check(self.ctx.lib.qk_sweep_compiled_multi(self.ctx.handle, module, len(progs), progs, *rest),
                       "qk_sweep_compiled_multi")

    def fuses_labels(self, fs) -> bool:
        return fs.dprog is not None and fs.dprog.module is not None

    def sweep_labels(self, fs, slot, sign, n_jobs, off, n_labels, q, ws, chunks=None):
        engine.sweep_labels(self.ctx, fs.dprog, slot, sign, n_jobs, off, n_labels, q=q, workspace=ws, chunks=chunks)

    def reduce_labels(self, pjob, off, n_labels, q):
        return engine.reduce_labels(self.ctx, pjob, off, n_labels, q=q)

    def gather_rows(self, q, idx, coef):
        return engine.gather_rows(self.ctx, q, idx, coef)

    def gemm_keyed(self, A, B, **kw):
        return engine.gemm_keyed(self.ctx, A, B, **kw)

    def khatri_rao(self, A, B):
        return engine.khatri_rao(self.ctx, A, B)

    def gemm_outer_paired(self, A, B, keyB, **kw):
        return engine.gemm_outer_paired(self.ctx, A, B, keyB, **kw)

    def knit_outer_stream(self, A, B, clbits_a, clbits_b, nbits, out, o_begin=0, o_count=None, k_dev=None):
        return engine.knit_outer_stream(self.ctx, A, B, clbits_a, clbits_b, nbits, out, o_begin=o_begin,
                                        o_count=o_count, k_dev=k_dev)

    def outer_stream_kernel(self, K, clbits_a, clbits_b, nbits, o_begin=0, o_count=None):
        return engine.knit_outer_stream_kernel(K, clbits_a, clbits_b, nbits, o_begin, o_count)

    def rank_factors(self, GA, GB):
        return engine.rank_factors_device(self.ctx, GA, GB)

    def prep_operands(self, WtA, qA, WtB, qB, probes):
        return engine.prep_operands(self.ctx, WtA, qA, WtB, qB, probes)

    fuses_tally = True

    def probe_errors(self, XA, A2, U, B2, probes, r=None, tol=0.0, a2_cols=None, rel_tol=0.0, tally=None, vpart=None):
        return engine.probe_errors(self.ctx, XA, A2, U, B2, probes, r=r, tol=tol, a2_cols=a2_cols, rel_tol=rel_tol,
                                   tally=tally, vpart=vpart)

    def compress_v(self, TA, XA, TB, XB, probes, a_cols=None, a_width=None):
        if os.environ.get("QKNIT_COMPRESS_V", "1") == "0" or not engine.compress_probe_v_ok(XA, XB, a_cols):
            return None
        return engine.compress_probe_v(self.ctx, TA, XA, TB, XB, probes, a_cols=a_cols, a_width=a_width)

    def probe_accept(self, e2, r, tol, rel_tol=0.0):
        return engine.probe_accept(self.ctx, e2, r, tol, rel_tol)

    def rank_tally(self, r, k, acc):
        self.ctx.check(self.ctx.lib.qk_rank_tally(self.ctx.handle, r.data_ptr(), k.data_ptr(), acc.data_ptr()),
                       "qk_rank_tally")

    def compress(self, TA, XA, TB, XB, a_cols=None, a_width=None):
        return engine.compress_operands(self.ctx, TA, XA, TB, XB, a_cols=a_cols, a_width=a_width)

    def knit_select(self, A, B, clbits_a, clbits_b, nbits, accuracy, k_dev=None):
        return engine.knit_select(self.ctx, A, B, clbits_a, clbits_b, nbits, accuracy, k_dev=k_dev)

    def npd_pairs(self, keys, vals):
        return engine.npd_pairs(self.ctx, keys, vals)

    def qprep_grams(self, WtA, qA, WtB, qB, probes):
        return engine.qprep_grams(self.ctx, WtA, qA, WtB, qB, probes)

    def qprep_compress_check(self, WtA, qA, WtB, qB, TA, TB, U, probes, r, tol, rel_tol):
        return engine.qprep_compress_check(self.ctx, WtA, qA, WtB, qB, TA, TB, U, probes, r, tol, rel_tol)

    def select_above(self, dense, accuracy, key_base=0):
        return engine.select_above(self.ctx, dense, accuracy, key_base=key_base)

    def npd_dense(self, dense, accuracy):
        return engine.nearest_probability_distribution(self.ctx, dense, accuracy)

    def out_buffer(self, n: int, select: bool = True):
        return engine.out_buffer(self.ctx, n, select=select)

    def event(self):
        return self.T.cuda.Event(enable_timing=True)


class KnitPipeline:
    def __init__(self, virt, device: int = 0, factored: bool = False, rank: int = 0, world: int = 1,
                 mode: str | None = None, group=None, backend=None, chunk_jobs: int | None = None,
                 jit: bool | None = None, light_cone: bool = True, data_rank: bool | None = None):
        self.be = backend if backend is not None else HipBackend(device)
        self.chunk_jobs = int(os.environ.get("QKNIT_SWEEP_CHUNK_JOBS", "0")) if chunk_jobs is None else chunk_jobs
        self.fork = False
        self._multi = None
        self._streams = []
        self._sweep_graph = None
        self.T = engine.torch()
        self.virt = virt
        self.rank, self.world, self.group = rank, world, group
        factored = factored and engine.factored_ok(virt)
        self.factored = factored
        kw = {} if light_cone else {"relevance": False}
        if jit is not None:
            kw["jit"] = jit
        self.plan_ms = {}
        tick = perf_counter()
        with engine.host_planning():
            self.frags = self.be.prepare_fragments(virt, basis=factored, **kw)
            tick = self._phase("prepare_fragments", tick)
            self.ops = engine.knit_operands(virt, self.frags, factored, compress=light_cone)
            tick = self._phase("knit_operands", tick)
        self.N = virt.circuit.num_clbits
        q_bytes = sum(len(fs.labels) << fs.prog.m for fs in self.frags) * 8
        out_bytes = (1 << self.N) * 8
        self.order = engine.contract_order(self.ops.clbits)
        if mode is None:
            if world == 1:
                mode = "single"
            elif out_bytes <= q_bytes and not factored:
                mode = "reduce"
            else:
                mode = "slice" if self.slice_ok(world) else "gather"
        if mode == "reduce" and factored:
            raise ValueError("reduce mode needs the direct (label-sliced) knit")
        if mode not in ("single", "reduce", "gather", "slice"):
            raise ValueError(f"unknown mode {mode}")
        if mode == "slice" and not self.slice_ok(world):
            raise ValueError("slice mode needs a factored two-fragment knit whose fragments partition the output "
                             "bits, a power-of-two world and >= 2^9 outputs per rank")
        self.mode = mode
        two = len(self.frags) == 2 and not any(fs.dropped for fs in self.frags)
        ok = mode in ("single", "gather", "slice") and factored and two
        self.data_rank = (ok and virt.circuit.num_clbits >= 24) if data_rank is None else (data_rank and ok)
        self.rank_tol = 1e-14
        self.rank_tol_rel = 1e-12
        self.rank_fallbacks = 0
        self.rank_incompressible = 0
        self.last_rank = None
        cA, cB = self._stream_bits()
        self.dev_rank = bool(self.data_rank and cA is not None and self.ops.num_terms <= 64
                             and hasattr(self.be, "rank_factors"))
        self._pending = 0
        self._tally = None
        self._tally_read = np.zeros(4, dtype=np.int64)
        self.slice_sync = os.environ.get("QKNIT_SLICE_SYNC", "0") == "1"
        self.slice_exact = os.environ.get("QKNIT_SLICE_EXACT", "predicated")
        self.last_kernel = None
        self.last_prep = None
        self._probe = None
        self._pinned = None
        self._prep_stream = None
        self._write_stream = None
        self.overlap_cus = None
        self.overlap = os.environ.get("QKNIT_OVERLAP", "0") == "1"
        self.spec_write = os.environ.get("QKNIT_SPEC_WRITE", "0") == "1"
        self._spec_stream = None
        ob = os.environ.get("QKNIT_OUT_BUFFERS", "")
        self.out_buffers = int(ob) if ob else (3 if world >= 8 else 2 if world >= 2 else 1)
        self._outs = None
        self._wstreams = None
        self._flip = 0
        self._write_cus = None
        self.events = []
        self.sweep_events = []
        self.prep_events = []
        self.record_events = False
        self.row_jobs = ROW_JOBS
        self.row_prune = ROW_PRUNE
        self.out_alloc = None
        self.slice_prep = None
        self.slice_costs = None
        self._plan()

    def _phase(self, name: str, since: float) -> float:
        now = perf_counter()
        self.plan_ms[name] = self.plan_ms.get(name, 0.0) + (now - since) * 1e3
        return now

    def _stream_bits(self):
        live = [i for i, fs in enumerate(self.frags) if not fs.dropped]
        if len(live) != 2 or len(self.order) != 2:
            return None, None
        cA, cB = self.ops.clbits[self.order[0]], self.ops.clbits[self.order[-1]]
        return (cA, cB) if engine.stream_knit_ok(cA, cB, self.N) else (None, None)

    def slice_ok(self, world: int) -> bool:
        cA, cB = self._stream_bits()
        if cA is None or world < 1 or world & (world - 1) or not self.factored:
            return False
        return (1 << self.N) // world >= 512 and min(len(cA), len(cB)) >= world.bit_length() - 1

    def _plan(self):
        T, be = self.T, self.be
        self.sweeps = []
        self.row_src, self.n_rows, self.plan_jobs = [], [], []
        L = self.ops.num_terms
        self.term_range = _shard(L, self.rank, self.world) if self.mode == "reduce" else (0, L)
        self.place = {}
# ... 310 lines not shown
    def _exchange(self, i, qpad):
        import torch.distributed as dist

        kind, send, recv = self.xbuf[i]
        if kind == "a2a":
            P, per, bw = send.shape
            send.copy_(qpad[:per].view(per, P, bw).transpose(0, 1))
            work = dist.all_to_all_single(recv, send, group=self.group, async_op=True)
        else:
            per = recv.shape[0] // self.world
            work = dist.all_gather_into_tensor(recv, qpad[:per], group=self.group, async_op=True)
        return work, recv

    def operands(self, qs: list) -> list:
        T, be = self.T, self.be
        mats = []
        for i, q in enumerate(qs):
            q = q.contiguous()
            if self.transforms[i] is not None:
                W = self.transforms[i]
                a = be.empty((W.shape[1], q.shape[1]), T.float64)
                be.gemm_keyed(W, q, out=a, strideA=q.shape[1])
            else:
                a = be.gather_rows(q, self.gather_idx[i], self.gather_coef[i])
            mats.append(a)
        return mats

    N_PROBES = 16
    RANK_GIVE_UP = 3

    def _probes(self, n: int, device):
        if self._probe is None or self._probe.shape[1] != n:
            key = (n, str(device))
            with _PROBES_LOCK:
                hit = _PROBES.get(key)
                if hit is None:
                    T = self.T
                    g = T.Generator().manual_seed(1234)
                    hit = _PROBES[key] = T.randn((self.N_PROBES, n), generator=g, dtype=T.float64).to(device)
            self._probe = hit
        return self._probe

    def _prep_step(self, qs) -> dict:
        return self._prep_slice(qs) if self.mode == "slice" and self.sharded else self._prep_dev_rank(qs)

    def _launch_step(self, p: dict):
        return self._launch_slice(p) if self.mode == "slice" else self._launch_dev_rank(p)

    def knit(self, qs: list):
        if self.dev_rank and self.mode in ("single", "slice"):
            p = self._prep_step(qs)
            if self.out is None:
                self.out = self._alloc_out(None)
            return self._launch_step(p)
        mats = self.operands(qs)
        if self.out is None:
            self.out = self._alloc_out(mats)
        if self.mode == "slice":
            ia, ib = self.order[0], self.order[-1]
            return self._slice_exact(mats[ia], mats[ib], self.ops.clbits[ia], self.ops.clbits[ib])
        low = self._rank_compress(mats) if self.data_rank else None
        if self.record_events:
            start, end = self.be.event(), self.be.event()
            start.record()
        if low is not None:
            res = self._contract_lowrank(low[0])
        elif self.mode == "single" and len(self.order) == 2 and mats[self.order[0]].shape[0] <= 8:
            res = self._contract_lowrank(mats)
        else:
            res = self._contract(mats)
        if self.record_events:
            end.record()
            self.events.append((start, end))
        if low is not None and not float(low[1]) <= max(self.rank_tol, self.rank_tol_rel * low[2]):
            self._rank_rejects = getattr(self, "_rank_rejects", 0) + 1
            if self._rank_rejects >= self.RANK_GIVE_UP:
                self.data_rank = False
            self.rank_fallbacks += 1
            self.last_rank = None
            res = self._contract(mats)
        elif low is not None:
            self._rank_rejects = 0
        if self.mode == "reduce":
            import torch.distributed as dist

            dist.reduce(res, dst=0, group=self.group)
        return res

    def _fused_prep(self, qs) -> bool:
        ia, ib = self.order[0], self.order[-1]
        if not hasattr(self.be, "prep_operands") or self.transforms[ia] is None or self.transforms[ib] is None:
            return False
        K = self.transforms[ia].shape[1]
        return (self.transforms[ib].shape[1] == K and self.transforms[ia].shape[0] == qs[ia].shape[0]
                and self.transforms[ib].shape[0] == qs[ib].shape[0]
                and engine.prep_ok(K, qs[ia].shape[1], qs[ib].shape[1]))

    def _qspace_prep(self, qs) -> bool:
        ia, ib = self.order[0], self.order[-1]
        if self.spec_write or not hasattr(self.be, "qprep_grams") or self.transforms[ia] is None \
                or self.transforms[ib] is None:
            return False
        WA, WB = self.transforms[ia], self.transforms[ib]
        return (WA.shape[1] == WB.shape[1] and WA.shape[0] == qs[ia].shape[0] and WB.shape[0] == qs[ib].shape[0]
                and engine.qprep_ok(WA.shape[1], WA.shape[0], WB.shape[0], qs[ia].shape[1], qs[ib].shape[1]))

    def _prep_fused(self, qs, probes):
        ia, ib = self.order[0], self.order[-1]
        qa = qs[ia] if qs[ia].stride(1) == 1 else qs[ia].contiguous()
        qb = qs[ib] if qs[ib].stride(1) == 1 else qs[ib].contiguous()
        XA, XB, G, U = self.be.prep_operands(self.transforms[ia], qa, self.transforms[ib], qb, probes)
        mats = [None] * len(qs)
        mats[ia], mats[ib] = XA, XB
        self.last_prep = "fused"
        return mats, G, U

    def _accept(self, A, B, A2, B2, x, r, ref_rows=None, cmp_rows=None, reduce_err=None, note=True):
        T = self.T
        if ref_rows is None:
            ref_rows = A.T @ _mm_nt(B, x)
            cmp_rows = A2.T @ _mm_nt(B2, x)
        e2 = T.cat([((ref_rows - cmp_rows) ** 2).sum(dim=0), (ref_rows ** 2).sum(dim=0)])
        if reduce_err is not None:
            e2 = reduce_err(e2)
        n = e2.numel() // 2
        err = e2[:n].max().sqrt()
        bound = T.clamp(self.rank_tol_rel * e2[n:].max().sqrt(), min=self.rank_tol)
        k_eff = T.where((err <= bound) & (r > 0), r, T.zeros_like(r))
        if note:
            self._note_rank(r, k_eff)
        return k_eff, err

    def _prep_dev_rank(self, qs) -> dict:
        ia, ib = self.order[0], self.order[-1]
        if self._qspace_prep(qs):
            T = self.T
            x = self._probes(qs[ib].shape[1], qs[ib].device)
            WA, WB = self.transforms[ia], self.transforms[ib]
            qA, qB = qs[ia].contiguous(), qs[ib].contiguous()
            G, U = self.be.qprep_grams(WA, qA, WB, qB, x)
            TA, TB, r = self.be.rank_factors(G[0], G[1])
            A2, B2, k_eff, _ = self.be.qprep_compress_check(WA, qA, WB, qB, TA, TB, U, x, r, self.rank_tol,
                                                            self.rank_tol_rel)
            self._note_rank(r, k_eff)
            mats = [None] * len(qs)
            for i, W, q in ((ia, WA, qA), (ib, WB, qB)):
                mats[i] = T.empty((W.shape[1], q.shape[1]), dtype=T.float64, device=q.device)
                self.be.gemm_keyed(W, q, out=mats[i], strideA=q.shape[1], skip=k_eff)
            self.last_prep = "qspace"
            return {"A2": A2, "B2": B2, "k_eff": k_eff, "mats": mats}
        if self._fused_prep(qs):
            x = self._probes(qs[ib].shape[1], qs[ib].device)
            mats, G, U = self._prep_fused(qs, x)
            TA, TB, r = self.be.rank_factors(G[0], G[1])
            if not self.spec_write:
                return self._compress_and_check(TA, TB, r, mats, U, x)
            A2, B2 = self.be.compress(TA, mats[ia], TB, mats[ib])
            if self.spec_write and getattr(self.be, "dev", None) is not None and self.be.dev.type == "cuda":
                T = self.T
                main = T.cuda.current_stream()
                if self._spec_stream is None:
                    self._spec_stream = T.cuda.Stream(device=self.be.dev)
                S2 = self._spec_stream
                S2.wait_stream(main)
                with T.cuda.stream(S2):
                    self.be.bind()
                    _, k_eff, _ = self.be.probe_errors(mats[ia], A2, U, B2, x, r=r, tol=self.rank_tol,
                                                       rel_tol=self.rank_tol_rel)
                    self._note_rank(r, k_eff)
                self.be.bind()
                for t in (mats[ia], A2, U, B2, x, r, k_eff):
                    t.record_stream(S2)
                return {"A2": A2, "B2": B2, "k_eff": k_eff, "k_write": r, "check": S2, "mats": mats}
            if getattr(self.be, "fuses_tally", False):
                _, k_eff, _ = self.be.probe_errors(mats[ia], A2, U, B2, x, r=r, tol=self.rank_tol,
                                                   rel_tol=self.rank_tol_rel, tally=self._tally_for(r.device))
                self._pending += 1
            else:
                _, k_eff, _ = self.be.probe_errors(mats[ia], A2, U, B2, x, r=r, tol=self.rank_tol,
                                                   rel_tol=self.rank_tol_rel)
                self._note_rank(r, k_eff)
            return {"A2": A2, "B2": B2, "k_eff": k_eff, "mats": mats}
        mats = self.operands(qs)
        self.last_prep = "torch"
        A, B = mats[ia], mats[ib]
        G = self.T.stack([_mm_nt(A, A), _mm_nt(B, B)])
        TA, TB, r = self.be.rank_factors(G[0].contiguous(), G[1].contiguous())
        A2, B2 = (TA @ A).contiguous(), (TB @ B).contiguous()
        k_eff, _ = self._accept(A, B, A2, B2, self._probes(B.shape[1], B.device), r)
        return {"A2": A2, "B2": B2, "k_eff": k_eff, "mats": mats}

    def _compress_and_check(self, TA, TB, r, mats, U, x) -> dict:
        ia, ib = self.order[0], self.order[-1]
        a_cols = self._replicated_a_cols()
        kw = {"a_cols": a_cols} if a_cols is not None else {}
        cv = self.be.compress_v(TA, mats[ia], TB, mats[ib], x, **kw) if hasattr(self.be, "compress_v") else None
        check = {}
        if cv is not None:
            A2, B2, check["vpart"] = cv
        else:
            A2, B2 = self.be.compress(TA, mats[ia], TB, mats[ib], **kw)
        XA = mats[ia]
        if a_cols is not None:
            XA = XA[:, a_cols[0]:a_cols[0] + a_cols[1]]
            check["a2_cols"] = a_cols
        tally = getattr(self.be, "fuses_tally", False)
        if tally:
            check["tally"] = self._tally_for(r.device)
        _, k_eff, _ = self.be.probe_errors(XA, A2, U, B2, x, r=r, tol=self.rank_tol, rel_tol=self.rank_tol_rel,
                                           **check)
        if tally:
            self._pending += 1
        else:
            self._note_rank(r, k_eff)
        return {"A2": A2, "B2": B2, "k_eff": k_eff, "mats": mats}

    def _kernel_name(self, K, cA, cB, o_begin=0, o_count=None):
        name = getattr(self.be, "outer_stream_kernel", None)
        return name(K, cA, cB, self.N, o_begin, o_count) if name else type(self.be).__name__

    def _launch_dev_rank(self, p: dict):
        ia, ib = self.order[0], self.order[-1]
        cA, cB = self.ops.clbits[ia], self.ops.clbits[ib]
        if self.record_events:
            start, end = self.be.event(), self.be.event()
            start.record()
        self.last_kernel = self._kernel_name(p["A2"].shape[0], cA, cB)
        self.be.knit_outer_stream(p["A2"], p["B2"], cA, cB, self.N, self.out, k_dev=p.get("k_write", p["k_eff"]))
        if self.record_events:
            end.record()
            self.events.append((start, end))
        if "check" in p:
            self.T.cuda.current_stream().wait_stream(p["check"])
        return self._contract(p["mats"], skip=p["k_eff"])

    def _prep_slice(self, qs) -> dict:
        import torch.distributed as dist

        T, be, P = self.T, self.be, self.world
        ia, ib = self.order[0], self.order[-1]
        bwA, bwB = qs[ia].shape[1], qs[ib].shape[1]
        x_full = self._probes(bwB * P, qs[ib].device)
        if getattr(self, "_x_local", None) is None or self._x_local.shape[1] != bwB:
            self._x_local = x_full[:, self.rank * bwB:(self.rank + 1) * bwB].contiguous()
        x = self._x_local
        npr = self.N_PROBES
        if self._fused_prep(qs):
            mats, G, U = self._prep_fused(qs, x)
            XA, XB = mats[ia], mats[ib]
            K = XA.shape[0]
            red = _joined(T, G, U)
            dist.all_reduce(red, group=self.group)
            G = red[:2 * K * K].view(2, K, K)
            U = red[2 * K * K:].view(K, npr).contiguous()
            TA, TB, r = be.rank_factors(G[0].contiguous(), G[1].contiguous())
            R8 = TA.shape[0]
            if self.slice_sync:
                fac = T.cat([TA.reshape(-1), TB.reshape(-1), r.to(T.float64)])
                dist.broadcast(fac, src=self._group_rank0(), group=self.group)
                TA = fac[:R8 * K].view(R8, K)
                TB = fac[R8 * K:2 * R8 * K].view(R8, K)
                r = fac[-1:].to(T.int32)
            A2l, B2l = be.compress(TA.contiguous(), XA, TB.contiguous(), XB)
            loc = _joined(T, A2l, B2l)
        else:
            mats = self.operands(qs)
            self.last_prep = "torch"
            XA, XB = mats[ia], mats[ib]
            K = XA.shape[0]
            red = T.cat([_mm_nt(XA, XA).reshape(-1), _mm_nt(XB, XB).reshape(-1), _mm_nt(XB, x).reshape(-1)])
            dist.all_reduce(red, group=self.group)
            GA = red[:K * K].view(K, K).contiguous()
            GB = red[K * K:2 * K * K].view(K, K).contiguous()
            Bx = red[2 * K * K:].view(K, npr)
            TA, TB, r = be.rank_factors(GA, GB)
            R8 = TA.shape[0]
            fac = T.cat([TA.reshape(-1), TB.reshape(-1), r.to(T.float64)])
            dist.broadcast(fac, src=self._group_rank0(), group=self.group)
            TA = fac[:R8 * K].view(R8, K)
            TB = fac[R8 * K:2 * R8 * K].view(R8, K)
            r = fac[-1:].to(T.int32)
            loc = T.cat([(TA @ XA).reshape(-1), (TB @ XB).reshape(-1)])
        gat = T.empty(P * loc.numel(), dtype=loc.dtype, device=loc.device)
        dist.all_gather_into_tensor(gat, loc, group=self.group)
        gat = gat.view(P, loc.numel())
        A2 = gat[:, :R8 * bwA].view(P, R8, bwA).permute(1, 0, 2).reshape(R8, P * bwA).contiguous()
        B2 = gat[:, R8 * bwA:].view(P, R8, bwB).permute(1, 0, 2).reshape(R8, P * bwB).contiguous()
        if self._fused_prep(qs):
            _, k_eff, _ = be.probe_errors(XA, A2, U, B2, x_full.contiguous(), r=r, tol=self.rank_tol,
                                          a2_cols=(self.rank * bwA, bwA), rel_tol=self.rank_tol_rel)
        else:
            ref_rows = XA.T @ Bx
            cmp_rows = A2[:, self.rank * bwA:(self.rank + 1) * bwA].T @ _mm_nt(B2, x_full)
            k_eff, _ = self._accept(None, None, None, None, None, r, ref_rows, cmp_rows, note=False)
        dist.all_reduce(k_eff, op=dist.ReduceOp.MIN, group=self.group)
        self._note_rank(r, k_eff)
        if self.slice_exact == "host":
            on_gpu = k_eff.device.type == "cuda"
            pinned = T.empty(1, dtype=T.int32, pin_memory=on_gpu)
            pinned.copy_(k_eff, non_blocking=on_gpu)
            ready = T.cuda.Event() if on_gpu else None
            if on_gpu:
                ready.record()
            return {"A2": A2, "B2": B2, "k_eff": k_eff, "XA": XA, "XB": XB, "pinned": pinned, "ready": ready,
                    "mats": mats}
        ex = self._slice_exact_operands(XA, XB, async_op=True)
        return {"A2": A2, "B2": B2, "k_eff": k_eff, "exact": ex, "mats": mats}

    def _launch_slice(self, p: dict):
        be = self.be
        ia, ib = self.order[0], self.order[-1]
        cA, cB = self.ops.clbits[ia], self.ops.clbits[ib]
        o_begin, o_count = self.slice
        if self.record_events:
            start, end = be.event(), be.event()
            start.record()
        self.last_kernel = self._kernel_name(p["A2"].shape[0], cA, cB, o_begin, o_count)
        be.knit_outer_stream(p["A2"], p["B2"], cA, cB, self.N, self.out, o_begin=o_begin, o_count=o_count,
                             k_dev=p["k_eff"])
        if self.record_events:
            end.record()
            self.events.append((start, end))
        if not self.sharded:
            if p.get("exact_queued"):
                return self.out
            A, kA, B, kB = self._slice_exact_operands(*self._exact_mats(p))
            be.gemm_keyed(A, B, keyA=kA, keyB=kB, out=self.out, skip=p["k_eff"])
            return self.out
        if "exact" not in p:
            if p["ready"] is not None:
                p["ready"].synchronize()
            if int(p["pinned"][0]) == 0:
                self._slice_exact(p["XA"], p["XB"], cA, cB)
            return self.out
        A, kA, B, kB = p["exact"]()
        be.gemm_keyed(A, B, keyA=kA, keyB=kB, out=self.out, skip=p["k_eff"])
        return self.out

    def overlap_ok(self) -> bool:
        return bool(self.dev_rank and self.mode in ("single", "slice") and getattr(self.be, "dev", None) is not None
                    and self.be.dev.type == "cuda")

    PREP_CUS = 96

    def _overlap_streams(self):
        if self._prep_stream is None:
            T = self.T
            dev = self.be.dev.index or 0
            env = os.environ.get("QKNIT_PREP_CUS", str(128 if self.world >= 4 else self.PREP_CUS))
            total = engine.device_cu_count(dev)
            if env == "all":
                every = tuple(range(total))
                self._prep_stream = engine.cu_masked_stream(dev, every)
                self._write_stream = engine.cu_masked_stream(dev, every, tag=100)
                self._write_cus = every
                self.overlap_cus = (total, total)
                self._prep_stream.wait_stream(T.cuda.current_stream())
                return self._prep_stream, self._write_stream
            c = int(env)
            if 0 < c < total:
                prep = tuple(range(total - c, total))
                write = tuple(i for i in range(total) if i not in set(prep))
                self._prep_stream = engine.cu_masked_stream(dev, prep)
                self._write_stream = engine.cu_masked_stream(dev, write)
                self._write_cus = write
                self.overlap_cus = (len(prep), len(write))
            else:
                prio = os.environ.get("QKNIT_OVERLAP_PRIO", "")
                hi = min(T.cuda.Stream.priority_range()) if prio else 0
                self._prep_stream = T.cuda.Stream(device=self.be.dev, priority=hi if prio == "prep" else 0)
                self._write_stream = T.cuda.Stream(device=self.be.dev, priority=hi) if prio == "write" else None
                self.overlap_cus = (0, total)
            self._prep_stream.wait_stream(T.cuda.current_stream())
        return self._prep_stream, self._write_stream

    def _step_overlapped(self):
        T, be = self.T, self.be
        main = T.cuda.current_stream()
        if main.cuda_stream == 0:
            raise ValueError("pipelined steps need a non-default current stream (torch.cuda.stream(...))")
        if self.out is None:
            return self.knit(self.sweep())
        S, W = self._overlap_streams()
        W = W if W is not None else main
        started = T.cuda.Event()
        started.record(main)
        self._started = (getattr(self, "_started", []) + [started])[-max(self.out_buffers, 1):]
        if self.out_buffers > 1:
            nb = self.out_buffers
            self._ensure_outs(W, main)
            k = self._flip
            self._flip = (self._flip + 1) % nb
            self.out, W = self._outs[k], self._wstreams[k]
        with T.cuda.stream(S):
            be.bind()
            if self.record_events:
                s0, s1 = be.event(), be.event()
                s0.record()
            qs = self.sweep()
            if self.record_events:
                s1.record()
                self.sweep_events.append((s0, s1))
            if self.out is None:
                self.out = self._alloc_out(None)
            p = self._prep_step(qs)
            if self._exact_before_write(W, main):
                if len(self._started) == max(self.out_buffers, 1):
                    S.wait_event(self._started[0])
                A, kA, B, kB = self._slice_exact_operands(*self._exact_mats(p))
                be.gemm_keyed(A, B, keyA=kA, keyB=kB, out=self.out, skip=p["k_eff"])
                p["exact_queued"] = True
            done = T.cuda.Event(enable_timing=self.record_events)
            done.record(S)
        if self.record_events:
            self.prep_events.append((s1, done))
        with T.cuda.stream(W):
            W.wait_event(done)
            if W is not main and len(self._started) == max(self.out_buffers, 1):
                W.wait_event(self._started[0])
            be.bind()
            for k in ("A2", "B2", "k_eff"):
                p[k].record_stream(W)
            for m in p["mats"]:
                if m is not None:
                    m.record_stream(W)
            out = self._launch_step(p)
        if W is not main:
            main.wait_stream(W)
        be.bind()
        return out

    def _replicated_a_cols(self):
        if self.mode != "slice" or self.sharded or self.spec_write or os.environ.get("QKNIT_SLICE_A_COLS") == "0":
            return None
        base, n = self._slice_exact_plan()[0][:2]
        width = 1 << len(self.ops.clbits[self.order[0]])
        return (base, n) if n < width and n % 16 == 0 else None

    def _ensure_outs(self, W, main) -> None:
        if self._outs is not None or self.out_buffers <= 1:
            return
        T, nb = self.T, self.out_buffers
        self._outs = [self.out] + [self._alloc_out(None) for _ in range(nb - 1)]
# ... 491 lines not shown
```

include/qknit.h:

```cpp
#ifndef QKNIT_H
#define QKNIT_H

#include <stdint.h>

#ifdef __cplusplus
extern "C" {
#endif

#define QK_OK 0
#define QK_EARG 1
#define QK_EHIP 2
#define QK_ESTATE 3

#define QK_TILE_BITS 12
#define QK_FIBER_BITS 4

enum { QK_U1 = 0, QK_D1 = 1, QK_SLOT = 2, QK_U2 = 3, QK_D2 = 4, QK_CX = 5, QK_SWAP = 6, QK_SCALE = 7,
       QK_U1R = 8, QK_U1X = 9, QK_D1R = 10, QK_D2R = 11, QK_SCALER = 12 };

typedef struct qk_op {
    int32_t kind;
    int32_t a, b;
    int32_t e1, e2;
    int32_t slot;
// ... 30 lines not shown
typedef struct qk_ctx qk_ctx;

int qk_ctx_create(int device, qk_ctx** out);
int qk_ctx_destroy(qk_ctx* ctx);
int qk_ctx_set_stream(qk_ctx* ctx, void* hip_stream);
int qk_ctx_synchronize(qk_ctx* ctx);
const char* qk_last_error(qk_ctx* ctx);

int qk_stream_create_cu_masked(int device, const uint32_t* cu_mask, int mask_words, void** stream);
int qk_stream_destroy(void* stream);
int qk_stream_cu_count(int device, void* stream, int* cus);
const char* qk_version(void);

int qk_out_alloc(qk_ctx* ctx, int64_t bytes, void** ptr);
int qk_out_free(qk_ctx* ctx, void* ptr);
int qk_out_mapped_bytes(const void* ptr, int64_t* bytes);
int qk_out_write_rate(qk_ctx* ctx, void* ptr, int64_t bytes, double* gbs);
int qk_out_stats(int64_t* out, int n);

int qk_sweep_workspace_bytes(const qk_program* prog, int64_t n_jobs, int64_t* bytes);

int qk_sweep(qk_ctx* ctx, const qk_program* prog, int64_t n_jobs, const double* job_slots,
             const double* job_sign, void* workspace, int64_t workspace_bytes, double* pjob);

typedef struct qk_module qk_module;

int qk_module_compile(qk_ctx* ctx, const char* source, const char* const* names, int n_names,
                      qk_module** out);
int qk_module_destroy(qk_module* module);
int qk_module_load(qk_ctx* ctx, const void* image, int64_t image_bytes, const char* const* names, int n_names,
                   qk_module** out);
int qk_module_code(const qk_module* module, void* buf, int64_t* bytes);

int qk_sweep_compiled(qk_ctx* ctx, const qk_module* module, const qk_program* prog, int64_t n_jobs,
                      const double* job_slots, const double* job_sign, void* workspace,
                      int64_t workspace_bytes, double* pjob);

int qk_sweep_compiled_labels(qk_ctx* ctx, const qk_module* module, const qk_program* prog, int64_t n_jobs,
                             const double* job_slots, const double* job_sign, int64_t n_labels,
                             const int64_t* label_offsets, void* workspace, int64_t workspace_bytes, double* q);

int qk_sweep_compiled_multi(qk_ctx* ctx, const qk_module* module, int n_prog, const qk_program* progs,
                            const int64_t* n_jobs, const double* const* job_slots, const double* const* job_sign,
                            const int64_t* n_labels, const int64_t* const* label_offsets, void* const* workspaces,
                            const int64_t* workspace_bytes, double* const* outs, const uint64_t* const* block_maps);

int qk_sweep_compiled_multi_shared(qk_ctx* ctx, const qk_module* module, int n_prog, const qk_program* progs,
                                   const int64_t* n_jobs, const double* const* job_slots,
                                   const double* const* job_sign, const int64_t* n_labels,
                                   const int64_t* const* label_offsets, void* const* workspaces,
                                   const int64_t* workspace_bytes, double* const* outs,
                                   const uint64_t* const* block_maps, const int64_t* n_init,
                                   const double* const* init_slots, const int32_t* const* prefix_of);

int qk_reduce_labels(qk_ctx* ctx, int64_t n_labels, const int64_t* offsets, int64_t width,
                     const double* pjob, double* q);

int qk_gemm_keyed(qk_ctx* ctx, int64_t M, int64_t N, int64_t K, const double* A, int64_t lda,
                  const double* B, int64_t ldb, const int64_t* keyA, int64_t strideA,
                  const int64_t* keyB, int64_t strideB, double* out, int beta);

int qk_gemm_keyed_pred(qk_ctx* ctx, int64_t M, int64_t N, int64_t K, const double* A, int64_t lda,
                       const double* B, int64_t ldb, const int64_t* keyA, int64_t strideA,
                       const int64_t* keyB, int64_t strideB, double* out, int beta, const int32_t* skip);

int qk_gemm_outer_paired(qk_ctx* ctx, int64_t M, int64_t N, int64_t K, const double* A, int64_t lda,
                         const double* B, int64_t ldb, const int64_t* keyA, int64_t strideA,
                         const int64_t* keyB, double* out);

int qk_knit_outer_stream(qk_ctx* ctx, int nbits, int64_t K, const double* A, int64_t lda, const double* B,
                         int64_t ldb, uint64_t maskA, uint64_t maskB, double* out);

int qk_knit_outer_stream_range(qk_ctx* ctx, int nbits, int64_t K, const double* A, int64_t lda, const double* B,
                               int64_t ldb, uint64_t maskA, uint64_t maskB, int64_t o_begin, int64_t o_count,
                               const int32_t* k_dev, double* out);

int qk_knit_outer_stream_kind(int nbits, int64_t K, uint64_t maskA, uint64_t maskB, int64_t o_begin,
                              int64_t o_count, int* kind, int* task_bits);
int qk_khatri_rao(qk_ctx* ctx, int64_t K, int64_t M, int64_t N, const double* A, int64_t lda,
                  const double* B, int64_t ldb, double* out);

int qk_gather_rows(qk_ctx* ctx, int64_t R, int64_t width, const int64_t* idx, const double* coef,
                   const double* src, double* dst);

typedef struct qk_knit_plan {
    int32_t n_frag;
    int32_t nbits;
    int64_t terms;
    const int64_t* rows;
    const uint64_t* clbit_masks;
    const double* const* transforms;
} qk_knit_plan;

int qk_knit_workspace_bytes(const qk_knit_plan* plan, int64_t* bytes);
int qk_knit(qk_ctx* ctx, const qk_knit_plan* plan, const double* const* q, void* workspace, int64_t workspace_bytes,
            double* out);

typedef struct qk_lowrank_plan {
    int32_t nbits;
    int32_t terms;
    int64_t rows_a, rows_b;
    uint64_t mask_a, mask_b;
    const double* wt_a;
    const double* wt_b;
    const double* probes;
    double lam_tol, s_tol, s_abs;
    double rank_tol;
    double rank_tol_rel;
} qk_lowrank_plan;

int qk_knit_lowrank_workspace_bytes(qk_ctx* ctx, const qk_lowrank_plan* plan, int64_t* bytes);
int qk_knit_lowrank(qk_ctx* ctx, const qk_lowrank_plan* plan, const double* q_a, const double* q_b, void* workspace,
                    int64_t workspace_bytes, double* out, int32_t* rank_out);

#define QK_COMM_ID_BYTES 128
typedef struct qk_comm qk_comm;
int qk_comm_unique_id(uint8_t* id);
int qk_comm_init(qk_ctx* ctx, const uint8_t* id, int nranks, int rank, qk_comm** out);
int qk_comm_destroy(qk_comm* comm);
int qk_comm_size(qk_comm* comm, int* nranks, int* rank);
int qk_allreduce(qk_ctx* ctx, qk_comm* comm, const double* send, double* recv, int64_t count);
int qk_reduce(qk_ctx* ctx, qk_comm* comm, const double* send, double* recv, int64_t count, int root);
int qk_allgather(qk_ctx* ctx, qk_comm* comm, const double* send, double* recv, int64_t count);
int qk_alltoall(qk_ctx* ctx, qk_comm* comm, const double* send, double* recv, int64_t count);

int qk_rank_factors(qk_ctx* ctx, int64_t K, const double* GA, const double* GB, double lam_tol, double s_tol,
                    double s_abs, int rmax, double* TA, double* TB, int32_t* r_out);

int qk_prep_workspace_bytes(qk_ctx* ctx, int64_t NA, int64_t NB, int64_t* bytes);
int qk_prep_operands(qk_ctx* ctx, int K, int RA, const double* WtA, const double* qA, int64_t ldqA, int64_t NA,
                     double* XA, int RB, const double* WtB, const double* qB, int64_t ldqB, int64_t NB, double* XB,
                     const double* probes, double* GA, double* GB, double* U, double* work, int64_t work_bytes);

int qk_qprep_workspace_bytes(qk_ctx* ctx, int64_t NA, int64_t NB, int64_t* bytes);
int qk_qprep_grams(qk_ctx* ctx, int K, int RA, const double* WtA, const double* qA, int64_t ldqA, int64_t NA, int RB,
                   const double* WtB, const double* qB, int64_t ldqB, int64_t NB, const double* probes, double* GA,
                   double* GB, double* U, double* work, int64_t work_bytes);
int qk_qprep_compress_check(qk_ctx* ctx, int K, int rmax, int RA, const double* WtA, const double* qA, int64_t ldqA,
                            int64_t NA, int RB, const double* WtB, const double* qB, int64_t ldqB, int64_t NB,
                            const double* TA, const double* TB, const double* U, const double* probes, double* A2,
                            double* B2, double* e2, const int32_t* r_dev, double tol, double rel_tol, int32_t* k_out,
                            double* err_out, double* work, int64_t work_bytes);

int qk_compress_operands(qk_ctx* ctx, int K, int rmax, const double* TA, const double* XA, int64_t NA, double* A2,
                         const double* TB, const double* XB, int64_t NB, double* B2);
int qk_compress_operands_ld(qk_ctx* ctx, int K, int rmax, const double* TA, const double* XA, int64_t NA, int64_t ldxa,
                            double* A2, int64_t lda2, const double* TB, const double* XB, int64_t NB, int64_t ldxb,
                            double* B2, int64_t ldb2);

int qk_compress_probe_v(qk_ctx* ctx, int K, int rmax, const double* TA, const double* XA, int64_t NA, int64_t ldxa,
                        double* A2, int64_t lda2, const double* TB, const double* XB, int64_t NB, int64_t ldxb,
                        double* B2, int64_t ldb2, const double* probes, int64_t ldp, double* vpart,
                        int64_t vpart_doubles);

int qk_probe_errors_vpart(qk_ctx* ctx, int K, int rmax, const double* XA, int64_t ldx, int64_t NA, const double* A2,
                          int64_t lda2, const double* U, const double* vpart, int64_t gv, double* e2,
                          const int32_t* r_dev, double tol, double rel_tol, int32_t* k_out, double* err_out,
                          double* work, int64_t work_bytes, int64_t* tally);

int qk_probe_workspace_bytes(qk_ctx* ctx, int64_t NA, int64_t* bytes);
int qk_probe_errors(qk_ctx* ctx, int K, int rmax, const double* XA, int64_t ldx, int64_t NA, const double* A2,
                    int64_t lda2, const double* U, const double* B2, int64_t ldb2, int64_t NB, const double* probes,
                    int64_t ldp, double* e2, const int32_t* r_dev, double tol, double rel_tol, int32_t* k_out,
                    double* err_out, double* work, int64_t work_bytes);
int qk_probe_errors_tally(qk_ctx* ctx, int K, int rmax, const double* XA, int64_t ldx, int64_t NA, const double* A2,
                          int64_t lda2, const double* U, const double* B2, int64_t ldb2, int64_t NB,
                          const double* probes, int64_t ldp, double* e2, const int32_t* r_dev, double tol,
                          double rel_tol, int32_t* k_out, double* err_out, double* work, int64_t work_bytes,
                          int64_t* tally);
int qk_probe_accept(qk_ctx* ctx, const double* e2, int n, const int32_t* r_dev, double tol, double rel_tol,
                    int32_t* k_out, double* err_out);
int qk_rank_tally(qk_ctx* ctx, const int32_t* r_dev, const int32_t* k_dev, int64_t* acc);


int qk_npd_workspace_bytes(int64_t n, int64_t count, int64_t* bytes);

int qk_threshold_count(qk_ctx* ctx, int64_t n, const double* vals, double acc, void* ws, int64_t ws_bytes,
                       int64_t* count_dev);

int qk_npd(qk_ctx* ctx, int64_t n, const double* vals, double acc, int64_t count, void* ws, int64_t ws_bytes,
           int64_t* out_keys, double* out_vals, int64_t* n_out_dev);

int qk_select_above(qk_ctx* ctx, int64_t n, const double* vals, double acc, int64_t key_base, int64_t capacity,
                    int64_t* keys, double* out_vals, int64_t* count_dev);


int qk_sample_cdf(qk_ctx* ctx, int64_t n_seg, const int64_t* seg_off, int64_t width, const double* pjob,
                  double* cdf);

int qk_sample_counts(qk_ctx* ctx, int64_t n_labels, int64_t label_base, const int64_t* label_seg,
                     const int64_t* seg_off, const int64_t* label_row_off, int64_t width, const double* cdf,
                     int64_t shots, uint64_t seed, unsigned int* counts);

int qk_fold_counts(qk_ctx* ctx, int64_t n_labels, const int64_t* label_row_off, int64_t width,
                   const double* row_sign, const unsigned int* counts, int64_t shots, double acc, double* q);

int qk_knit_select_workspace_bytes(int nbits, uint64_t maskA, uint64_t maskB, int64_t* bytes);
int qk_knit_select(qk_ctx* ctx, int nbits, int64_t K, const double* A, int64_t lda, const double* B, int64_t ldb,
                   uint64_t maskA, uint64_t maskB, double acc, const int32_t* k_dev, void* work, int64_t work_bytes,
                   int64_t capacity, int64_t* keys, double* vals, int64_t* count_dev);

int qk_npd_pairs_workspace_bytes(int64_t count, int64_t* bytes);
int qk_npd_pairs(qk_ctx* ctx, int64_t count, const int64_t* keys, const double* vals, void* ws, int64_t ws_bytes,
                 int64_t* out_keys, double* out_vals, int64_t* n_out_dev);

int qk_qd_from_rows(qk_ctx* ctx, int64_t n_rows, int64_t width, const double* rows, const int64_t* dst, double acc,
                    double* out);
int qk_qd_merge(qk_ctx* ctx, int64_t na, const double* a, const int64_t* ka, int64_t nb, const double* b,
                const int64_t* kb, double acc, int64_t n_out, double* out);
int qk_qd_axpby(qk_ctx* ctx, int64_t n, double alpha, const double* a, double beta, const double* b, double acc,
                double* out);

int qk_hellinger(qk_ctx* ctx, int64_t n, const double* p, const double* q, double* acc3);

#ifdef __cplusplus
}
#endif
#endif
```

Before: 522,800.

## Overlap probe reference product with rank factorization and add prep tail rows

```diff
diff --git a/hardwareawareoptimalquantumcircuitcuttingandknitting_amd/_lib.py b/hardwareawareoptimalquantumcircuitcuttingandknitting_amd/_lib.py
--- a/hardwareawareoptimalquantumcircuitcuttingandknitting_amd/_lib.py
+++ b/hardwareawareoptimalquantumcircuitcuttingandknitting_amd/_lib.py
@@ -97,6 +97,12 @@
     "qk_probe_errors_vpart": (c_i32, [c_vp, ctypes.c_int, ctypes.c_int, c_vp, c_i64, c_i64, c_vp, c_i64, c_vp, c_vp,
                                       c_i64, c_vp, c_vp, ctypes.c_double, ctypes.c_double, c_vp, c_vp, c_vp, c_i64,
                                       c_vp]),
+    "qk_rank_factors_ref": (c_i32, [c_vp, c_i64, c_vp, c_vp, ctypes.c_double, ctypes.c_double, ctypes.c_double,
+                                    ctypes.c_int, c_vp, c_vp, c_vp, c_vp, c_i64, c_i64, c_vp, c_vp, c_i64]),
+    "qk_probe_ref_workspace_bytes": (c_i32, [c_vp, c_i64, ctypes.POINTER(c_i64), ctypes.POINTER(c_i64)]),
+    "qk_probe_errors_ref": (c_i32, [c_vp, ctypes.c_int, c_i64, c_vp, c_i64, c_vp, c_i64, c_vp, c_i64, c_i64, c_vp,
+                                    c_i64, c_vp, c_vp, ctypes.c_double, ctypes.c_double, c_vp, c_vp, c_vp, c_i64,
+                                    c_vp]),
     "qk_probe_workspace_bytes": (c_i32, [c_vp, c_i64, ctypes.POINTER(c_i64)]),
     "qk_probe_errors": (c_i32, [c_vp, ctypes.c_int, ctypes.c_int, c_vp, c_i64, c_i64, c_vp, c_i64, c_vp, c_vp, c_i64,
                                 c_i64, c_vp, c_i64, c_vp, c_vp, ctypes.c_double, ctypes.c_double, c_vp, c_vp, c_vp,
diff --git a/hardwareawareoptimalquantumcircuitcuttingandknitting_amd/csrc/qknit_prep.hip b/hardwareawareoptimalquantumcircuitcuttingandknitting_amd/csrc/qknit_prep.hip
--- a/hardwareawareoptimalquantumcircuitcuttingandknitting_amd/csrc/qknit_prep.hip
+++ b/hardwareawareoptimalquantumcircuitcuttingandknitting_amd/csrc/qknit_prep.hip
@@ -1,6 +1,7 @@
 #include <hip/hip_runtime.h>
 
 #include <cstdint>
+#include <cstdlib>
 #include <string>
 
 #include "internal.h"
@@ -65,14 +66,20 @@
 #endif
 constexpr int QLD = PCT + QK_PREP_QPAD;
 constexpr int WLD = PK + QK_PREP_WPAD;
+constexpr int PTR = 4;
+template <bool TAIL>
 struct PrepStage {
-    double q[PRS][QLD];
-    double w[PRS][WLD];
+    double q[PRS + (TAIL ? PTR : 0)][QLD];
+    double w[PRS + (TAIL ? PTR : 0)][WLD];
 };
+template <bool TAIL>
 union PrepLds {
-    PrepStage st[PNS];
+    PrepStage<TAIL> st[PNS];
     double x[PK][XLD];
 };
+static_assert(sizeof(PrepLds<true>) * QK_PREP_WG_PER_CU <= 160 * 1024,
+              "the stage ring with remainder rows must leave QK_PREP_WG_PER_CU workgroups resident per CU (160 KiB of LDS)");
+__host__ __device__ constexpr bool prep_tail(int R) { return R > PRS && R % PRS >= 1 && R % PRS <= PTR; }
 
 __device__ __forceinline__ void prep_glds(const double* src, double* lds_row) {
     __builtin_amdgcn_global_load_lds(reinterpret_cast<const void*>(src),
@@ -90,8 +97,9 @@
     }
 }
 
+template <bool TAIL>
 __global__ __launch_bounds__(PTH, 2 * QK_PREP_WG_PER_CU) void qk_prep_operands_kernel(PrepArgs a) {
-    __shared__ __attribute__((aligned(16))) PrepLds L;
+    __shared__ __attribute__((aligned(16))) PrepLds<TAIL> L;
     const int tid = threadIdx.x, lane = tid & 63, wave = tid >> 6;
     const int l16 = lane & 15, l4 = lane >> 4;
     const int K = a.K;
@@ -109,7 +117,8 @@
     for (int sd = 0; sd < 2; ++sd) {
         const PrepSide& S = a.s[sd];
         const int R = S.R;
-        const int nst = (R + PRS - 1) / PRS;
+        const bool tail = TAIL && prep_tail(R);
+        const int nst = tail ? R / PRS : (R + PRS - 1) / PRS;
         const int64_t tiles = S.N / PCT;
         d4_t g0 = {0, 0, 0, 0}, g1 = {0, 0, 0, 0}, u = {0, 0, 0, 0};
         const bool mine = !a.split || (int)(blockIdx.x & 1) == sd;
@@ -119,11 +128,20 @@
             const int64_t c0 = t * PCT;
             int nload[PNS];
             auto issue = [&](int st) {
-                PrepStage& P = L.st[st % PNS];
+                PrepStage<TAIL>& P = L.st[st % PNS];
                 int n = 0;
 #pragma unroll
                 for (int h = 0; h < PRPW; ++h) {
                     const int rl = PRPW * wave_s + h, r = st * PRS + rl;
+                    if (r < R) {
+                        prep_glds(S.q + (int64_t)r * S.ldq + c0 + 2 * lane, &P.q[rl][0]);
+                        ++n;
+                        if (2 * lane < K) prep_glds(S.Wt + (int64_t)r * K + 2 * lane, &P.w[rl][0]);
+                        ++n;
+                    }
+                }
+                if (TAIL && tail && st == nst - 1 && wave_s < PTR) {
+                    const int rl = PRS + wave_s, r = st * PRS + rl;
                     if (r < R) {
                         prep_glds(S.q + (int64_t)r * S.ldq + c0 + 2 * lane, &P.q[rl][0]);
                         ++n;
@@ -145,7 +163,7 @@
                 prep_vmwait(after);
                 asm volatile("s_waitcnt lgkmcnt(0)" ::: "memory");
                 __builtin_amdgcn_s_barrier();
-                const PrepStage& P = L.st[st % PNS];
+                const PrepStage<TAIL>& P = L.st[st % PNS];
                 double qb[PRS / 4], wa[PRS / 4][4];
 #pragma unroll
                 for (int kk = 0; kk < PRS / 4; ++kk) {
@@ -163,6 +181,19 @@
                 for (int kk = 0; kk < PRS / 4; ++kk)
 #pragma unroll
                     for (int i = 0; i < 4; ++i) x[i] = __builtin_amdgcn_mfma_f64_16x16x4f64(wa[kk][i], qb[kk], x[i], 0, 0, 0);
+                if (TAIL && tail && st == nst - 1) {
+                    const int rl = PRS + l4;
+                    const bool rv = st * PRS + rl < R;
+                    const double qe = rv ? P.q[rl][16 * wave + l16] : 0.0;
+                    double we[4];
+#pragma unroll
+                    for (int i = 0; i < 4; ++i) {
+                        const int k = 16 * i + l16;
+                        we[i] = (rv && k < K) ? P.w[rl][k] : 0.0;
+                    }
+#pragma unroll
+                    for (int i = 0; i < 4; ++i) x[i] = __builtin_amdgcn_mfma_f64_16x16x4f64(we[i], qe, x[i], 0, 0, 0);
+                }
             }
             const bool probes = S.P != nullptr && wave < 4;
             constexpr int PPB = 8;
@@ -657,6 +688,74 @@
         epart[(int64_t)blockIdx.x * 2 * PNP + tid] = ep[0][tid] + ep[1][tid] + ep[2][tid] + ep[3][tid];
 }
 
+__global__ __launch_bounds__(256) void qk_probe_dref_kernel(int rmax, const double* __restrict__ racc, int64_t NA,
+                                                            const double* __restrict__ A2, int64_t lda2,
+                                                            const double* __restrict__ vpart, int gv,
+                                                            double* __restrict__ epart) {
+    __shared__ double Vs[16][PNP];
+    __shared__ double ep[4][2 * PNP];
+    const int tid = threadIdx.x, lane = tid & 63, wave = tid >> 6, l16 = lane & 15, l4 = lane >> 4;
+    int64_t cb = (int64_t)blockIdx.x * 4 + wave;
+    const int64_t step = (int64_t)gridDim.x * 4, nblk = NA / 16;
+    d4_t acc = {0, 0, 0, 0};
+    double a2[2] = {0.0, 0.0};
+    auto fetch = [&](int64_t b) {
+        const int64_t bl = b < nblk ? b : nblk - 1;
+        acc = *reinterpret_cast<const d4_t*>(racc + bl * 256 + 4 * lane);
+#pragma unroll
+        for (int jj = 0; jj < 2; ++jj) a2[jj] = A2[(int64_t)min(4 * jj + l4, rmax - 1) * lda2 + bl * 16 + l16];
+    };
+    fetch(cb);
+    {
+        __shared__ double vh[PV_PART];
+        const int e = tid & (PV_PART - 1), h = tid >> 7;
+        double t[16];
+#pragma unroll
+        for (int u = 0; u < 16; ++u) t[u] = 0.0;
+        int b = h;
+        for (; b + 30 < gv; b += 32) {
+            double v[16];
+#pragma unroll
+            for (int u = 0; u < 16; ++u) v[u] = vpart[(int64_t)(b + 2 * u) * PV_PART + e];
+#pragma unroll
+            for (int u = 0; u < 16; ++u) t[u] += v[u];
+        }
+        for (; b < gv; b += 2) t[0] += vpart[(int64_t)b * PV_PART + e];
+#pragma unroll
+        for (int w = 8; w >= 1; w >>= 1)
+#pragma unroll
+            for (int u = 0; u < w; ++u) t[u] += t[u + w];
+        if (h == 1) vh[e] = t[0];
+        __syncthreads();
+        if (h == 0) Vs[e / 16][e % 16] = -(t[0] + vh[e]);
+        else Vs[8 + e / 16][e % 16] = 0.0;
+    }
+    __syncthreads();
+    double e2 = 0.0, f2 = 0.0;
+    for (; cb < nblk; cb += step) {
+        d4_t d = acc;
+        const double b0 = a2[0], b1 = a2[1];
+        fetch(cb + step);
+#pragma unroll
+        for (int rr = 0; rr < 4; ++rr) f2 = fma(d[rr], d[rr], f2);
+        d = __builtin_amdgcn_mfma_f64_16x16x4f64(b0, Vs[l4][l16], d, 0, 0, 0);
+        d = __builtin_amdgcn_mfma_f64_16x16x4f64(b1, Vs[4 + l4][l16], d, 0, 0, 0);
+#pragma unroll
+        for (int rr = 0; rr < 4; ++rr) e2 = fma(d[rr], d[rr], e2);
+    }
+    e2 += __shfl_xor(e2, 16, 64);
+    e2 += __shfl_xor(e2, 32, 64);
+    f2 += __shfl_xor(f2, 16, 64);
+    f2 += __shfl_xor(f2, 32, 64);
+    if (l4 == 0) {
+        ep[wave][l16] = e2;
+        ep[wave][PNP + l16] = f2;
+    }
+    __syncthreads();
+    if (tid < 2 * PNP)
+        epart[(int64_t)blockIdx.x * 2 * PNP + tid] = ep[0][tid] + ep[1][tid] + ep[2][tid] + ep[3][tid];
+}
+
 constexpr int PE = 2 * PNP;
 
 __global__ __launch_bounds__(256) void qk_probe_accept_kernel(const double* __restrict__ epart, int n,
@@ -1163,6 +1262,8 @@
 bool prep_split(qk_ctx* ctx, int64_t NA, int64_t NB) {
     const int64_t tiles = (NA > NB ? NA : NB) / PCT;
     const int64_t g = (int64_t)(ctx->cus > 0 ? ctx->cus : 256) * QK_PREP_WG_PER_CU;
+    const char* env = getenv("QKNIT_PREP_SPLIT");
+    if (env && atoi(env) == 0) return false;
     return QK_PREP_SPLIT && tiles > 0 && 2 * tiles <= g;
 }
 
@@ -1206,7 +1307,11 @@
     args.K = K;
     args.split = prep_split(ctx, NA, NB) ? 1 : 0;
     args.part = work;
-    hipLaunchKernelGGL(qk_prep_operands_kernel, dim3(G), dim3(PTH), 0, ctx->stream, args);
+    const char* tail_env = getenv("QKNIT_PREP_TAIL");
+    if ((prep_tail(RA) || prep_tail(RB)) && !(tail_env && atoi(tail_env) == 0))
+        hipLaunchKernelGGL(qk_prep_operands_kernel<true>, dim3(G), dim3(PTH), 0, ctx->stream, args);
+    else
+        hipLaunchKernelGGL(qk_prep_operands_kernel<false>, dim3(G), dim3(PTH), 0, ctx->stream, args);
     const int outs = 2 * PPG + PNP * K;
     hipLaunchKernelGGL(qk_prep_reduce_kernel, dim3((outs + 63) / 64), dim3(64 * PRW), 0, ctx->stream, work, G, K, GA,
                        GB, U);
@@ -1386,6 +1491,47 @@
     return QK_OK;
 }
 
+int qk_probe_ref_workspace_bytes(qk_ctx* ctx, int64_t NA, int64_t* bytes, int64_t* acc_offset) {
+    if (!ctx || !bytes || !acc_offset || NA < 0) return QK_EARG;
+    *acc_offset = (int64_t)PV_GRID * PV_PART + (int64_t)probe_grid_d(ctx, NA) * PE;
+    *bytes = (*acc_offset + NA * 16) * (int64_t)sizeof(double);
+    return QK_OK;
+}
+
+int qk_probe_errors_ref(qk_ctx* ctx, int rmax, int64_t NA, const double* A2, int64_t lda2, const double* vpart,
+                        int64_t gv, const double* B2, int64_t ldb2, int64_t NB, const double* probes, int64_t ldp,
+                        double* e2, const int32_t* r_dev, double tol, double rel_tol, int32_t* k_out, double* err_out,
+                        double* work, int64_t work_bytes, int64_t* tally) {
+    if (!ctx) return QK_EARG;
+    if (rmax < 1 || rmax > 8 || NA < 16 || NA % 16 || lda2 < NA)
+        return fail(ctx, QK_EARG, "qk_probe_errors_ref: need 1 <= rmax <= 8, NA % 16 == 0, lda2 >= NA");
+    if (!A2 || !work || (k_out && !r_dev) || (tally && !k_out))
+        return fail(ctx, QK_EARG, "qk_probe_errors_ref: null buffer");
+    if (vpart ? gv < 1 : (!B2 || !probes || NB < 4 || NB % 4 || ldb2 < NB || ldp < NB))
+        return fail(ctx, QK_EARG, "qk_probe_errors_ref: need V partials (gv >= 1) or B2 and the probes (NB % 4 == 0)");
+    int64_t need = 0, off = 0;
+    qk_probe_ref_workspace_bytes(ctx, NA, &need, &off);
+    if (work_bytes < need || (reinterpret_cast<uintptr_t>(work) & 31))
+        return fail(ctx, QK_EARG, "qk_probe_errors_ref: workspace too small or not 32-B aligned (qk_probe_ref_workspace_bytes)");
+    if (hipSetDevice(ctx->device) != hipSuccess) return fail(ctx, QK_EHIP, "qk_probe_errors_ref: hipSetDevice");
+    const int gd = probe_grid_d(ctx, NA);
+    double* epart = work + PV_GRID * PV_PART;
+    if (!vpart) {
+        hipLaunchKernelGGL(qk_probe_v_kernel, dim3(PV_GRID), dim3(256), 0, ctx->stream, rmax, B2, ldb2, NB, probes, ldp,
+                           work);
+        vpart = work;
+        gv = PV_GRID;
+    }
+    hipLaunchKernelGGL(qk_probe_dref_kernel, dim3(gd), dim3(256), 0, ctx->stream, rmax, work + off, NA, A2, lda2, vpart,
+                       (int)gv, epart);
+    hipLaunchKernelGGL(qk_probe_accept_kernel, dim3(1), dim3(256), 0, ctx->stream, epart, gd, r_dev, tol, rel_tol, e2,
+                       k_out, err_out, tally);
+    const hipError_t e = hipGetLastError();
+    if (e != hipSuccess)
+        return fail(ctx, QK_EHIP, (std::string("qk_probe_errors_ref: ") + hipGetErrorString(e)).c_str());
+    return QK_OK;
+}
+
 int qk_probe_errors(qk_ctx* ctx, int K, int rmax, const double* XA, int64_t ldx, int64_t NA, const double* A2,
                     int64_t lda2, const double* U, const double* B2, int64_t ldb2, int64_t NB, const double* probes,
                     int64_t ldp, double* e2, const int32_t* r_dev, double tol, double rel_tol, int32_t* k_out,
diff --git a/hardwareawareoptimalquantumcircuitcuttingandknitting_amd/csrc/qknit_rank.hip b/hardwareawareoptimalquantumcircuitcuttingandknitting_amd/csrc/qknit_rank.hip
--- a/hardwareawareoptimalquantumcircuitcuttingandknitting_amd/csrc/qknit_rank.hip
+++ b/hardwareawareoptimalquantumcircuitcuttingandknitting_amd/csrc/qknit_rank.hip
@@ -97,7 +97,7 @@
     idx = bi;
 }
 
-__global__ __launch_bounds__(RK_THREADS) void qk_rank_factors_kernel(RankArgs a) {
+__device__ __forceinline__ void rank_factors_body(const RankArgs& a) {
     __shared__ double G[2][RK_K][RK_K + 1];
     __shared__ double L[2][RK_K][RK_RC + 1];
     __shared__ double C[RK_RC][RK_RC + 1];
@@ -257,6 +257,54 @@
 #endif
 }
 
+__global__ __launch_bounds__(RK_THREADS) void qk_rank_factors_kernel(RankArgs a) { rank_factors_body(a); }
+
+typedef double rk_d4_t __attribute__((ext_vector_type(4)));
+constexpr int RK_NP = 16;
+
+struct RefArgs {
+    const double* XA;
+    int64_t ldx, NA;
+    const double* U;
+    double* acc;
+};
+
+__global__ __launch_bounds__(RK_THREADS) void qk_rank_factors_ref_kernel(RankArgs a, RefArgs f) {
+    if (blockIdx.x == 0) {
+        rank_factors_body(a);
+        return;
+    }
+    __shared__ double Us[RK_K][RK_NP];
+    const int tid = threadIdx.x, lane = tid & 63, wave = tid >> 6, l16 = lane & 15, l4 = lane >> 4, K = a.K;
+    const int64_t nblk = f.NA / 16;
+    const int64_t w0 = (int64_t)(blockIdx.x - 1) * 2 + wave, nw = (int64_t)(gridDim.x - 1) * 2;
+    auto fetch = [&](int64_t cb, double (&av)[RK_K / 4]) {
+        const int64_t c = (cb < nblk ? cb : nblk - 1) * 16 + l16;
+#pragma unroll
+        for (int kk = 0; kk < RK_K / 4; ++kk) av[kk] = f.XA[(int64_t)min(4 * kk + l4, K - 1) * f.ldx + c];
+    };
+    auto mac = [&](int64_t cb, const double (&av)[RK_K / 4]) {
+        rk_d4_t acc = {0, 0, 0, 0};
+#pragma unroll
+        for (int kk = 0; kk < RK_K / 4; ++kk)
+            acc = __builtin_amdgcn_mfma_f64_16x16x4f64(av[kk], Us[4 * kk + l4][l16], acc, 0, 0, 0);
+        *reinterpret_cast<rk_d4_t*>(f.acc + cb * 256 + 4 * lane) = acc;
+    };
+    double x0[RK_K / 4], x1[RK_K / 4];
+    if (w0 < nblk) fetch(w0, x0);
+    for (int e = tid; e < RK_K * RK_NP; e += RK_THREADS) Us[e / RK_NP][e % RK_NP] = (e / RK_NP) < K ? f.U[e] : 0.0;
+    __syncthreads();
+    for (int64_t cb = w0; cb < nblk; cb += 2 * nw) {
+        fetch(cb + nw, x1);
+        __builtin_amdgcn_sched_barrier(0);
+        mac(cb, x0);
+        if (cb + nw >= nblk) break;
+        fetch(cb + 2 * nw, x0);
+        __builtin_amdgcn_sched_barrier(0);
+        mac(cb + nw, x1);
+    }
+}
+
 }
 
 #ifdef QK_RANK_DEBUG
@@ -289,3 +337,38 @@
     }
     return QK_OK;
 }
+
+extern "C" int qk_rank_factors_ref(qk_ctx* ctx, int64_t K, const double* GA, const double* GB, double lam_tol,
+                                   double s_tol, double s_abs, int rmax, double* TA, double* TB, int32_t* r_out,
+                                   const double* XA, int64_t ldx, int64_t NA, const double* U, double* acc,
+                                   int64_t acc_doubles) {
+    if (!ctx) return QK_EARG;
+    if (K < 1 || K > RK_K || rmax < 1 || rmax > RK_R || NA < 16 || NA % 16 || ldx < NA) {
+        ctx->err = "qk_rank_factors_ref: need 1 <= K <= 64, 1 <= rmax <= 8, NA % 16 == 0, ldx >= NA";
+        return QK_EARG;
+    }
+    if (!GA || !GB || !TA || !TB || !r_out || !XA || !U || !acc) {
+        ctx->err = "qk_rank_factors_ref: null buffer";
+        return QK_EARG;
+    }
+    if (acc_doubles < NA * 16 || (reinterpret_cast<uintptr_t>(acc) & 31)) {
+        ctx->err = "qk_rank_factors_ref: accumulator store too small or not 32-B aligned (qk_probe_ref_workspace_bytes)";
+        return QK_EARG;
+    }
+    if (hipSetDevice(ctx->device) != hipSuccess) {
+        ctx->err = "qk_rank_factors_ref: hipSetDevice";
+        return QK_EHIP;
+    }
+    const int cap = (ctx->cus > 0 ? ctx->cus : 256) - 1;
+    const int g = cap > 1 ? cap : 1;
+    RankArgs args{(int)K, rmax, GA, GB, lam_tol, s_tol, s_abs, TA, TB, r_out};
+    RefArgs ref{XA, ldx, NA, U, acc};
+    hipLaunchKernelGGL(qk_rank_factors_ref_kernel, dim3((unsigned)(1 + g)), dim3(RK_THREADS), 0, ctx->stream, args,
+                       ref);
+    const hipError_t e = hipGetLastError();
+    if (e != hipSuccess) {
+        ctx->err = std::string("qk_rank_factors_ref: ") + hipGetErrorString(e);
+        return QK_EHIP;
+    }
+    return QK_OK;
+}
diff --git a/hardwareawareoptimalquantumcircuitcuttingandknitting_amd/engine.py b/hardwareawareoptimalquantumcircuitcuttingandknitting_amd/engine.py
--- a/hardwareawareoptimalquantumcircuitcuttingandknitting_amd/engine.py
+++ b/hardwareawareoptimalquantumcircuitcuttingandknitting_amd/engine.py
@@ -959,6 +959,38 @@
     return TA, TB, r
 
 
+_PROBE_REF_WORK: dict = {}
+
+
+def probe_ref_ok(XA) -> bool:
+    return XA.shape[1] >= 16 and XA.shape[1] % 16 == 0 and XA.stride(1) == 1 and XA.stride(0) >= XA.shape[1]
+
+
+def rank_factors_ref_device(ctx: Context, GA, GB, XA, U, rmax: int = 8):
+    from . import data_rank as dr
+
+    T = torch()
+    K, NA = XA.shape
+    assert GA.shape == (K, K) and GB.shape == (K, K) and GA.is_contiguous() and GB.is_contiguous()
+    assert U.shape == (K, N_PROBES) and U.is_contiguous() and probe_ref_ok(XA)
+    dev = XA.device
+    need, off = ctypes.c_int64(), ctypes.c_int64()
+    ctx.check(ctx.lib.qk_probe_ref_workspace_bytes(ctx.handle, NA, ctypes.byref(need), ctypes.byref(off)),
+              "qk_probe_ref_workspace_bytes")
+    key = (str(dev), T.cuda.current_stream(dev).cuda_stream)
+    work = _PROBE_REF_WORK.get(key)
+    if work is None or work.numel() * 8 < need.value:
+        work = _PROBE_REF_WORK[key] = T.empty(max(need.value // 8, 1), dtype=T.float64, device=dev)
+    TA = T.empty((rmax, K), dtype=T.float64, device=dev)
+    TB = T.empty((rmax, K), dtype=T.float64, device=dev)
+    r = T.empty(1, dtype=T.int32, device=dev)
+    ctx.check(ctx.lib.qk_rank_factors_ref(ctx.handle, K, GA.data_ptr(), GB.data_ptr(), dr.LAM_TOL, dr.S_TOL, dr.S_ABS,
+                                          rmax, TA.data_ptr(), TB.data_ptr(), r.data_ptr(), XA.data_ptr(),
+                                          XA.stride(0), NA, U.data_ptr(), work.data_ptr() + 8 * off.value,
+                                          work.numel() - off.value), "qk_rank_factors_ref")
+    return TA, TB, r, (work, NA)
+
+
 PREP_COLS = 128
 N_PROBES = 16
 _PREP_WORK: dict = {}
@@ -1120,7 +1152,7 @@
 
 _PROBE_WORK: dict = {}
 def probe_errors(ctx: Context, XA, A2, U, B2, probes, r=None, tol: float = 0.0, a2_cols: tuple | None = None,
-                 rel_tol: float = 0.0, tally=None, vpart=None):
+                 rel_tol: float = 0.0, tally=None, vpart=None, ref=None):
     T = torch()
     K, NA = XA.shape
     rmax = A2.shape[0]
@@ -1131,16 +1163,25 @@
     off = 0 if a2_cols is None else a2_cols[0]
     assert (a2_cols is None and A2.shape[1] == NA) or (a2_cols is not None and a2_cols[1] == NA)
     dev = XA.device
+    e2 = T.empty(2 * N_PROBES, dtype=T.float64, device=dev)
+    k = T.empty(1, dtype=T.int32, device=dev) if r is not None else None
+    err = T.empty(1, dtype=T.float64, device=dev) if r is not None else None
+    assert tally is None or (r is not None and tally.dtype == T.int64 and tally.numel() == 4)
+    if ref is not None:
+        work, ref_na = ref
+        assert ref_na == NA and (vpart is None or (vpart.is_contiguous() and vpart.shape[1:] == (8, N_PROBES)))
+        ctx.check(ctx.lib.qk_probe_errors_ref(ctx.handle, rmax, NA, A2.data_ptr() + 8 * off, A2.shape[1], _ptr(vpart),
+                                              0 if vpart is None else vpart.shape[0], B2.data_ptr(), NB, NB,
+                                              probes.data_ptr(), NB, e2.data_ptr(), _ptr(r), tol, rel_tol, _ptr(k),
+                                              _ptr(err), work.data_ptr(), work.numel() * 8, _ptr(tally)),
+                  "qk_probe_errors_ref")
+        return e2, k, err
     need = ctypes.c_int64()
     ctx.check(ctx.lib.qk_probe_workspace_bytes(ctx.handle, NA, ctypes.byref(need)), "qk_probe_workspace_bytes")
     key = (str(dev), T.cuda.current_stream(dev).cuda_stream)
     work = _PROBE_WORK.get(key)
     if work is None or work.numel() * 8 < need.value:
         work = _PROBE_WORK[key] = T.empty(max(need.value // 8, 1), dtype=T.float64, device=dev)
-    e2 = T.empty(2 * N_PROBES, dtype=T.float64, device=dev)
-    k = T.empty(1, dtype=T.int32, device=dev) if r is not None else None
-    err = T.empty(1, dtype=T.float64, device=dev) if r is not None else None
-    assert tally is None or (r is not None and tally.dtype == T.int64 and tally.numel() == 4)
     if vpart is not None:
         assert vpart.is_contiguous() and vpart.shape[1:] == (8, N_PROBES)
         ctx.check(ctx.lib.qk_probe_errors_vpart(ctx.handle, K, rmax, XA.data_ptr(), XA.stride(0), NA,
diff --git a/hardwareawareoptimalquantumcircuitcuttingandknitting_amd/pipeline.py b/hardwareawareoptimalquantumcircuitcuttingandknitting_amd/pipeline.py
--- a/hardwareawareoptimalquantumcircuitcuttingandknitting_amd/pipeline.py
+++ b/hardwareawareoptimalquantumcircuitcuttingandknitting_amd/pipeline.py
@@ -264,14 +264,20 @@
     def rank_factors(self, GA, GB):
         return engine.rank_factors_device(self.ctx, GA, GB)
 
+    def rank_factors_ref(self, GA, GB, XA, U):
+        if os.environ.get("QKNIT_PROBE_REF", "1") == "0" or not engine.probe_ref_ok(XA):
+            return (*engine.rank_factors_device(self.ctx, GA, GB), None)
+        return engine.rank_factors_ref_device(self.ctx, GA, GB, XA, U)
+
     def prep_operands(self, WtA, qA, WtB, qB, probes):
         return engine.prep_operands(self.ctx, WtA, qA, WtB, qB, probes)
 
     fuses_tally = True
 
-    def probe_errors(self, XA, A2, U, B2, probes, r=None, tol=0.0, a2_cols=None, rel_tol=0.0, tally=None, vpart=None):
+    def probe_errors(self, XA, A2, U, B2, probes, r=None, tol=0.0, a2_cols=None, rel_tol=0.0, tally=None, vpart=None,
+                     ref=None):
         return engine.probe_errors(self.ctx, XA, A2, U, B2, probes, r=r, tol=tol, a2_cols=a2_cols, rel_tol=rel_tol,
-                                   tally=tally, vpart=vpart)
+                                   tally=tally, vpart=vpart, ref=ref)
 
     def compress_v(self, TA, XA, TB, XB, probes, a_cols=None, a_width=None):
         if os.environ.get("QKNIT_COMPRESS_V", "1") == "0" or not engine.compress_probe_v_ok(XA, XB, a_cols):
@@ -888,9 +894,10 @@
         if self._fused_prep(qs):
             x = self._probes(qs[ib].shape[1], qs[ib].device)
             mats, G, U = self._prep_fused(qs, x)
+            if not self.spec_write:
+                TA, TB, r, ref = self._factors_and_ref(G[0], G[1], self._check_columns(mats[ia]), U)
+                return self._compress_and_check(TA, TB, r, mats, U, x, ref=ref)
             TA, TB, r = self.be.rank_factors(G[0], G[1])
-            if not self.spec_write:
-                return self._compress_and_check(TA, TB, r, mats, U, x)
             A2, B2 = self.be.compress(TA, mats[ia], TB, mats[ib])
             if self.spec_write and getattr(self.be, "dev", None) is not None and self.be.dev.type == "cuda":
                 T = self.T
@@ -926,7 +933,16 @@
         k_eff, _ = self._accept(A, B, A2, B2, self._probes(B.shape[1], B.device), r)
         return {"A2": A2, "B2": B2, "k_eff": k_eff, "mats": mats}
 
-    def _compress_and_check(self, TA, TB, r, mats, U, x) -> dict:
+    def _check_columns(self, XA):
+        a_cols = self._replicated_a_cols()
+        return XA if a_cols is None else XA[:, a_cols[0]:a_cols[0] + a_cols[1]]
+
+    def _factors_and_ref(self, GA, GB, XA, U):
+        if hasattr(self.be, "rank_factors_ref"):
+            return self.be.rank_factors_ref(GA, GB, XA, U)
+        return (*self.be.rank_factors(GA, GB), None)
+
+    def _compress_and_check(self, TA, TB, r, mats, U, x, ref=None) -> dict:
         ia, ib = self.order[0], self.order[-1]
         a_cols = self._replicated_a_cols()
         kw = {"a_cols": a_cols} if a_cols is not None else {}
@@ -936,10 +952,11 @@
             A2, B2, check["vpart"] = cv
         else:
             A2, B2 = self.be.compress(TA, mats[ia], TB, mats[ib], **kw)
-        XA = mats[ia]
+        XA = self._check_columns(mats[ia])
         if a_cols is not None:
-            XA = XA[:, a_cols[0]:a_cols[0] + a_cols[1]]
             check["a2_cols"] = a_cols
+        if ref is not None:
+            check["ref"] = ref
         tally = getattr(self.be, "fuses_tally", False)
         if tally:
             check["tally"] = self._tally_for(r.device)
@@ -989,7 +1006,7 @@
             dist.all_reduce(red, group=self.group)
             G = red[:2 * K * K].view(2, K, K)
             U = red[2 * K * K:].view(K, npr).contiguous()
-            TA, TB, r = be.rank_factors(G[0].contiguous(), G[1].contiguous())
+            TA, TB, r, ref = self._factors_and_ref(G[0].contiguous(), G[1].contiguous(), XA, U)
             R8 = TA.shape[0]
             if self.slice_sync:
                 fac = T.cat([TA.reshape(-1), TB.reshape(-1), r.to(T.float64)])
@@ -1023,8 +1040,9 @@
         A2 = gat[:, :R8 * bwA].view(P, R8, bwA).permute(1, 0, 2).reshape(R8, P * bwA).contiguous()
         B2 = gat[:, R8 * bwA:].view(P, R8, bwB).permute(1, 0, 2).reshape(R8, P * bwB).contiguous()
         if self._fused_prep(qs):
+            check = {"ref": ref} if ref is not None else {}
             _, k_eff, _ = be.probe_errors(XA, A2, U, B2, x_full.contiguous(), r=r, tol=self.rank_tol,
-                                          a2_cols=(self.rank * bwA, bwA), rel_tol=self.rank_tol_rel)
+                                          a2_cols=(self.rank * bwA, bwA), rel_tol=self.rank_tol_rel, **check)
         else:
             ref_rows = XA.T @ Bx
             cmp_rows = A2[:, self.rank * bwA:(self.rank + 1) * bwA].T @ _mm_nt(B2, x_full)
diff --git a/include/qknit.h b/include/qknit.h
--- a/include/qknit.h
+++ b/include/qknit.h
@@ -206,6 +206,15 @@
                         double* A2, int64_t lda2, const double* TB, const double* XB, int64_t NB, int64_t ldxb,
                         double* B2, int64_t ldb2, const double* probes, int64_t ldp, double* vpart,
                         int64_t vpart_doubles);
+
+int qk_rank_factors_ref(qk_ctx* ctx, int64_t K, const double* GA, const double* GB, double lam_tol, double s_tol,
+                        double s_abs, int rmax, double* TA, double* TB, int32_t* r_out, const double* XA, int64_t ldx,
+                        int64_t NA, const double* U, double* acc, int64_t acc_doubles);
+int qk_probe_ref_workspace_bytes(qk_ctx* ctx, int64_t NA, int64_t* bytes, int64_t* acc_offset);
+int qk_probe_errors_ref(qk_ctx* ctx, int rmax, int64_t NA, const double* A2, int64_t lda2, const double* vpart,
+                        int64_t gv, const double* B2, int64_t ldb2, int64_t NB, const double* probes, int64_t ldp,
+                        double* e2, const int32_t* r_dev, double tol, double rel_tol, int32_t* k_out, double* err_out,
+                        double* work, int64_t work_bytes, int64_t* tally);
 
 int qk_probe_errors_vpart(qk_ctx* ctx, int K, int rmax, const double* XA, int64_t ldx, int64_t NA, const double* A2,
                           int64_t lda2, const double* U, const double* vpart, int64_t gv, double* e2,
```

Result: no change. 522,800 (-0.0%).
